# facebookresearch/SlowFast

Measured on NVIDIA H100. Metric: clips/sec (fwd+bwd) SlowFast-8x8-R50, higher is better.
Workload: dtype bf16x3-split operands, f32 accumulate/storage

## Files before the change

slowfast_b200/csrc/conv_stem.cu:

```cuda
#include <algorithm>
#include <cstdint>
#include <cstring>
#include <cuda_bf16.h>

#include "../../include/slowfast_b200.h"
#include "ptx.cuh"
#include "tmap.h"

namespace sfb {

constexpr int ST_MAX_STAGES = 8;
constexpr int ST_SEG_STRIDE = 2304;
constexpr int ST_SEG_PIX = 136;
constexpr int ST_WSEG_STRIDE = 1152;
constexpr int ST_WSEG_PIX = 72;
constexpr int ST_MMA_WARPS = 8;
constexpr int ST_FPROP_THREADS = 32 * (ST_MMA_WARPS + 1 + 4);
constexpr int ST_WGRAD_THREADS = 32 * (4 + 1);
constexpr int ST_BN_MAX = 128;
constexpr int ST_NPG_MAX = 4;

__device__ __forceinline__ void tma_load_5d(void* smem, const CUtensorMap* tm, uint64_t* bar, int32_t c0, int32_t c1,
                                            int32_t c2, int32_t c3, int32_t c4) {
  asm volatile(
      "cp.async.bulk.tensor.5d.shared::cluster.global.mbarrier::complete_tx::bytes [%0], [%1, {%3, %4, %5, %6, %7}], "
      "[%2];" ::"r"(smem_u32(smem)),
      "l"(tm), "r"(smem_u32(bar)), "r"(c0), "r"(c1), "r"(c2), "r"(c3), "r"(c4)
      : "memory");
}
__device__ __forceinline__ void tma_load_3d_(void* smem, const CUtensorMap* tm, uint64_t* bar, int32_t c0, int32_t c1,
                                             int32_t c2) {
  asm volatile(
      "cp.async.bulk.tensor.3d.shared::cluster.global.mbarrier::complete_tx::bytes [%0], [%1, {%3, %4, %5}], [%2];"
      ::"r"(smem_u32(smem)), "l"(tm), "r"(smem_u32(bar)), "r"(c0), "r"(c1), "r"(c2)
      : "memory");
}

struct StemParams {
  CUtensorMap tmX[2];
  CUtensorMap tmB[2];
  int N, OT, OH, OW;
  int st, sh, pt, ph, pw;
  int KT, KH, KW;
  int pairs, pps, k_blocks;
  int cout, BN, w_tiles, m_tiles;
  int stages;
  uint32_t stage_bytes, a_plane_bytes, b_bytes;
  uint32_t acc_pitch, off_acc, off_staging, off_red, off_bars;
  float* out;
  float* stats;
  int npg, n_groups, co_tiles, ktot, kb_total, splits, kb_per_split, w_chunks;
  float* dw;
};

template <int NSPLIT>
__global__ void __launch_bounds__(ST_FPROP_THREADS, 1) stem_fprop_kernel(const __grid_constant__ StemParams p) {
  extern __shared__ uint8_t smem_raw[];
  uint8_t* smem = reinterpret_cast<uint8_t*>((reinterpret_cast<uintptr_t>(smem_raw) + 1023) & ~uintptr_t(1023));
  const int warp = threadIdx.x >> 5, lane = threadIdx.x & 31;
  uint64_t* full = reinterpret_cast<uint64_t*>(smem + p.off_bars);
  uint64_t* empty = full + ST_MAX_STAGES;
  uint64_t* tfull = empty + ST_MAX_STAGES;
  uint64_t* tempty = tfull + 1;
  float* acc_tile = reinterpret_cast<float*>(smem + p.off_acc);
  if (threadIdx.x == 0) {
    for (int s = 0; s < p.stages; ++s) {
      mbar_init(&full[s], 1);
      mbar_init(&empty[s], 32 * ST_MMA_WARPS);
    }
    mbar_init(tfull, 32 * ST_MMA_WARPS);
    mbar_init(tempty, 4);
    fence_mbar_init();
    fence_proxy_async_smem();
  }
  __syncthreads();
  constexpr uint32_t NP = NSPLIT == 3 ? 2u : 1u;
  const int total_tiles = p.m_tiles;
  const int ksteps_per_pair = p.KW / 2;

  if (warp == ST_MMA_WARPS) {
    int stage = 0;
    uint32_t phase = 0;
    for (int tile = blockIdx.x; tile < total_tiles; tile += gridDim.x) {
      const int wt = tile % p.w_tiles;
      int r = tile / p.w_tiles;
      const int oh = r % p.OH;
      r /= p.OH;
      const int ot = r % p.OT;
      const int n = r / p.OT;
      const int w0 = wt * 128 - p.pw;
      for (int kb = 0; kb < p.k_blocks; ++kb) {
        mbar_wait(&empty[stage], phase ^ 1);
        if (elect_one()) {
          const int pair0 = kb * p.pps;
          const int nq = min(p.pps, p.pairs - pair0);
          mbar_expect_tx(&full[stage], (uint32_t(nq) * ST_SEG_PIX * 16u + p.b_bytes) * NP);
          uint8_t* st = smem + size_t(stage) * p.stage_bytes;
          for (int qq = 0; qq < nq; ++qq) {
            const int pair = pair0 + qq;
            const int kt = pair / p.KH, kh = pair - kt * p.KH;
            const int h = oh * p.sh - p.ph + kh, t = ot * p.st - p.pt + kt;
            for (uint32_t pl = 0; pl < NP; ++pl)
              tma_load_5d(st + pl * p.a_plane_bytes + qq * ST_SEG_STRIDE, &p.tmX[pl], &full[stage], 0, w0, h, t, n);
          }
          for (uint32_t pl = 0; pl < NP; ++pl)
            tma_load_2d(st + NP * p.a_plane_bytes + pl * p.b_bytes, &p.tmB[pl], &full[stage], kb * 64, 0);
        }
        __syncwarp();
        if (++stage == p.stages) {
          stage = 0;
          phase ^= 1;
        }
      }
    }
  } else if (warp < ST_MMA_WARPS) {
    const int g = warp >> 2;
    float d[ST_BN_MAX / 2];
    int stage = 0;
    uint32_t phase = 0;
    int it = 0;
    for (int tile = blockIdx.x; tile < total_tiles; tile += gridDim.x, ++it) {
      int held = -1;
      for (int kb = 0; kb < p.k_blocks; ++kb) {
        mbar_wait(&full[stage], phase);
        wgmma_fence();
        const int nq = min(p.pps, p.pairs - kb * p.pps);
        const uint32_t a_base = smem_u32(smem + size_t(stage) * p.stage_bytes) + uint32_t(g) * 1024u;
        const uint32_t b_base = smem_u32(smem + size_t(stage) * p.stage_bytes) + NP * p.a_plane_bytes;
        int kstep = 0;
        for (int qq = 0; qq < nq; ++qq) {
          for (int j = 0; j < ksteps_per_pair; ++j, ++kstep) {
            const uint32_t aa = a_base + qq * ST_SEG_STRIDE + uint32_t(2 * j) * 16u;
            const uint64_t a_hi = make_smem_desc(aa, 16, 128, 0);
            const uint64_t b_hi = make_smem_desc(b_base + uint32_t(kstep) * 32u, 16, 1024, 2);
            const uint32_t acc_flag = (kb | kstep) != 0 ? 1u : 0u;
            if (NSPLIT == 3) {
              const uint64_t a_lo = make_smem_desc(aa + p.a_plane_bytes, 16, 128, 0);
              const uint64_t b_lo = make_smem_desc(b_base + p.b_bytes + uint32_t(kstep) * 32u, 16, 1024, 2);
              wgmma_bf16<ST_BN_MAX, 0, 0>(d, p.BN, a_lo, b_hi, acc_flag);
              wgmma_bf16<ST_BN_MAX, 0, 0>(d, p.BN, a_hi, b_lo, 1u);
              wgmma_bf16<ST_BN_MAX, 0, 0>(d, p.BN, a_hi, b_hi, 1u);
            } else {
              wgmma_bf16<ST_BN_MAX, 0, 0>(d, p.BN, a_hi, b_hi, acc_flag);
            }
          }
        }
        wgmma_commit();
        wgmma_wait<1>();
        if (held >= 0) mbar_arrive(&empty[held]);
        held = stage;
        if (++stage == p.stages) {
          stage = 0;
          phase ^= 1;
        }
      }
      wgmma_wait<0>();
      mbar_arrive(&empty[held]);
      mbar_wait(tempty, (it & 1) ^ 1);
      acc_store<ST_BN_MAX>(d, p.BN, acc_tile + size_t(g) * 64 * p.acc_pitch, int(p.acc_pitch));
      mbar_arrive(tfull);
    }
  } else {
    const int q = warp - (ST_MMA_WARPS + 1);
    float* stg = reinterpret_cast<float*>(smem + p.off_staging) + q * (32 * 33);
    float* red = reinterpret_cast<float*>(smem + p.off_red);
    const float* arow = acc_tile + size_t(q * 32 + lane) * p.acc_pitch;
    int it = 0;
    for (int tile = blockIdx.x; tile < total_tiles; tile += gridDim.x, ++it) {
      const int acc = it & 1;
      const int wt = tile % p.w_tiles;
      const int rowi = tile / p.w_tiles;
      const int ow = wt * 128 + q * 32 + lane;
      const bool rvalid = ow < p.OW;
      const uint32_t rmask = __ballot_sync(0xffffffffu, rvalid);
      float* red_w = red + ((size_t(acc) * 4 + q) * p.BN) * 2;
      mbar_wait(tfull, it & 1);
      for (int c0 = 0; c0 < p.BN; c0 += 32) {
        uint32_t v0[16], v1[16];
        acc_ld_x16(arow + c0, v0);
        const bool second = (c0 + 16) < p.BN;
        if (second) acc_ld_x16(arow + c0 + 16, v1);
        if (c0 + 32 >= p.BN) {
          __syncwarp();
          if (lane == 0) mbar_arrive(tempty);
        }
#pragma unroll
        for (int j = 0; j < 16; ++j) stg[lane * 33 + j] = rvalid ? __uint_as_float(v0[j]) : 0.f;
#pragma unroll
        for (int j = 0; j < 16; ++j) stg[lane * 33 + 16 + j] = (rvalid && second) ? __uint_as_float(v1[j]) : 0.f;
        __syncwarp();
        {
          const int cl = c0 + lane;
          const bool cvalid = cl < min(p.BN, p.cout);
          float* dst = p.out + (static_cast<long long>(rowi) * p.OW + wt * 128 + q * 32) * p.cout + cl;
          if (p.cout <= 16 && (p.cout & (p.cout - 1)) == 0 && p.BN <= 32) {
            const int W = p.cout;
            const int R = 32 / W;
            const int col = lane & (W - 1), rsub = lane / W;
            float s = 0.f, s2 = 0.f;
            float* d2 = p.out + (static_cast<long long>(rowi) * p.OW + wt * 128 + q * 32) * p.cout + col;
            for (int r0 = 0; r0 < 32; r0 += R) {
              const int r = r0 + rsub;
              const float y = stg[r * 33 + col];
              s += y;
              s2 = fmaf(y, y, s2);
              if ((rmask >> r) & 1u) d2[static_cast<long long>(r) * p.cout] = y;
            }
            for (int o = W; o < 32; o <<= 1) {
              s += __shfl_xor_sync(0xffffffffu, s, o);
              s2 += __shfl_xor_sync(0xffffffffu, s2, o);
            }
            if (p.stats != nullptr && lane < W) {
              red_w[lane * 2 + 0] = s;
              red_w[lane * 2 + 1] = s2;
            }
            if (p.stats != nullptr && lane >= W && lane < p.BN) {
              red_w[lane * 2 + 0] = 0.f;
              red_w[lane * 2 + 1] = 0.f;
            }
            __syncwarp();
            continue;
          }
          float s = 0.f, s2 = 0.f;
#pragma unroll 8
          for (int r = 0; r < 32; ++r) {
            const float y = stg[r * 33 + lane];
            s += y;
            s2 = fmaf(y, y, s2);
            if (((rmask >> r) & 1u) && cvalid) dst[static_cast<long long>(r) * p.cout] = y;
          }
          if (p.stats != nullptr && cl < p.BN) {
            red_w[cl * 2 + 0] = s;
            red_w[cl * 2 + 1] = s2;
          }
          __syncwarp();
        }
      }
      if (p.stats != nullptr) {
        named_bar_sync(1, 128);
        const float* rb = red + size_t(acc) * 4 * p.BN * 2;
        for (int cl = q * 32 + lane; cl < p.BN; cl += 128) {
          if (cl < p.cout) {
            float s = 0.f, s2 = 0.f;
#pragma unroll
            for (int w = 0; w < 4; ++w) {
              s += rb[(size_t(w) * p.BN + cl) * 2 + 0];
              s2 += rb[(size_t(w) * p.BN + cl) * 2 + 1];
            }
            p.stats[size_t(cl) * p.m_tiles + tile] = s;
            p.stats[(size_t(p.cout) + cl) * p.m_tiles + tile] = s2;
          }
        }
      }
    }
  }
}

__device__ __forceinline__ void st_red_add_v4(float* addr, float a, float b, float c, float d) {
  asm volatile("red.global.add.v4.f32 [%0], {%1, %2, %3, %4};" ::"l"(addr), "f"(a), "f"(b), "f"(c), "f"(d)
               : "memory");
}

template <int NSPLIT>
__global__ void __launch_bounds__(ST_WGRAD_THREADS, 1) stem_wgrad_kernel(const __grid_constant__ StemParams p) {
  extern __shared__ uint8_t smem_raw[];
  uint8_t* smem = reinterpret_cast<uint8_t*>((reinterpret_cast<uintptr_t>(smem_raw) + 1023) & ~uintptr_t(1023));
  const int warp = threadIdx.x >> 5, lane = threadIdx.x & 31;
  uint64_t* full = reinterpret_cast<uint64_t*>(smem + p.off_bars);
  uint64_t* empty = full + ST_MAX_STAGES;
  constexpr uint32_t NP = NSPLIT == 3 ? 2u : 1u;

  const int split = blockIdx.x % p.splits;
  const int grp = blockIdx.x / p.splits;
  const int kb0 = split * p.kb_per_split;
  const int kb1 = min(p.kb_total, kb0 + p.kb_per_split);
  const int pair_base = grp * p.npg;
  const int npairs = min(p.npg, p.pairs - pair_base);
  const int ncols_pair = p.KW * 8;

  if (threadIdx.x == 0) {
    for (int s = 0; s < p.stages; ++s) {
      mbar_init(&full[s], 1);
      mbar_init(&empty[s], 128);
    }
    fence_mbar_init();
    fence_proxy_async_smem();
  }
  __syncthreads();
  const uint32_t dy_plane = 8192;

  if (kb1 > kb0 && npairs > 0) {
    if (warp == 4) {
      int stage = 0;
      uint32_t phase = 0;
      for (int kb = kb0; kb < kb1; ++kb) {
        mbar_wait(&empty[stage], phase ^ 1);
        if (elect_one()) {
          const int wc = kb % p.w_chunks;
          int r = kb / p.w_chunks;
          const int rowi = r;
          const int oh = r % p.OH;
          r /= p.OH;
          const int ot = r % p.OT;
          const int n = r / p.OT;
          const int ow0 = wc * 64;
          mbar_expect_tx(&full[stage], (dy_plane + uint32_t(npairs) * ST_WSEG_PIX * 16u) * NP);
          uint8_t* st = smem + size_t(stage) * p.stage_bytes;
          for (uint32_t pl = 0; pl < NP; ++pl) {
            tma_load_3d_(st + pl * dy_plane, &p.tmB[pl], &full[stage], 0, ow0, rowi);
            uint8_t* xb = st + NP * dy_plane + pl * p.a_plane_bytes;
            for (int j = 0; j < npairs; ++j) {
              const int pair = pair_base + j;
              const int kt = pair / p.KH, kh = pair - kt * p.KH;
              tma_load_5d(xb + j * ST_WSEG_STRIDE, &p.tmX[pl], &full[stage], 0, ow0 - p.pw, oh * p.sh - p.ph + kh,
                          ot * p.st - p.pt + kt, n);
            }
          }
        }
        __syncwarp();
        if (++stage == p.stages) {
          stage = 0;
          phase ^= 1;
        }
      }
    } else {
      float d[ST_NPG_MAX * 16];
      int stage = 0;
      uint32_t phase = 0;
      int held = -1;
      for (int kb = kb0; kb < kb1; ++kb) {
        mbar_wait(&full[stage], phase);
        wgmma_fence();
        const uint32_t a_base = smem_u32(smem + size_t(stage) * p.stage_bytes);
        const uint32_t x_base = a_base + NP * dy_plane;
#pragma unroll
        for (int j = 0; j < ST_NPG_MAX; ++j) {
          if (j < npairs) {
#pragma unroll
            for (int ks = 0; ks < 4; ++ks) {
              const uint64_t a_hi = make_smem_desc(a_base + ks * 2048, 0, 1024, 2);
              const uint64_t b_hi = make_smem_desc(x_base + j * ST_WSEG_STRIDE + ks * 256, 128, 16, 0);
              const uint32_t acc_flag = (kb != kb0 || ks != 0) ? 1u : 0u;
              if (NSPLIT == 3) {
                const uint64_t a_lo = make_smem_desc(a_base + dy_plane + ks * 2048, 0, 1024, 2);
                const uint64_t b_lo =
                    make_smem_desc(x_base + p.a_plane_bytes + j * ST_WSEG_STRIDE + ks * 256, 128, 16, 0);
                wgmma_bf16<32, 1, 1>(d + 16 * j, ncols_pair, a_lo, b_hi, acc_flag);
                wgmma_bf16<32, 1, 1>(d + 16 * j, ncols_pair, a_hi, b_lo, 1u);
                wgmma_bf16<32, 1, 1>(d + 16 * j, ncols_pair, a_hi, b_hi, 1u);
              } else {
                wgmma_bf16<32, 1, 1>(d + 16 * j, ncols_pair, a_hi, b_hi, acc_flag);
              }
            }
          }
        }
        wgmma_commit();
        wgmma_wait<1>();
        if (held >= 0) mbar_arrive(&empty[held]);
        held = stage;
        if (++stage == p.stages) {
          stage = 0;
          phase ^= 1;
        }
      }
      wgmma_wait<0>();
      const int co0 = warp * 16 + (lane >> 2);
      const int col_base = pair_base * ncols_pair;
#pragma unroll
      for (int j = 0; j < ST_NPG_MAX; ++j) {
        if (j < npairs) {
#pragma unroll
          for (int c = 0; c < 4; ++c) {
            if (8 * c < ncols_pair) {
#pragma unroll
              for (int h = 0; h < 2; ++h) {
                const int co = co0 + 8 * h;
                if (co < p.cout) {
                  float* dst = p.dw + size_t(co) * p.ktot + col_base + j * ncols_pair + 8 * c + 2 * (lane & 3);
                  asm volatile("red.global.add.v2.f32 [%0], {%1, %2};" ::"l"(dst), "f"(d[16 * j + 4 * c + 2 * h]),
                               "f"(d[16 * j + 4 * c + 2 * h + 1]) : "memory");
                }
              }
            }
          }
        }
      }
    }
  }
}

__global__ void stem_input_fold_kernel(const float* __restrict__ x, int n, int cin, int t, int h, int w,
                                       __nv_bfloat16* __restrict__ hi, __nv_bfloat16* __restrict__ lo) {
  const int w2 = w / 2;
  const int64_t thw = int64_t(t) * h * w;
  const int64_t items = int64_t(n) * t * h * w2;
  for (int64_t i = blockIdx.x * int64_t(blockDim.x) + threadIdx.x; i < items; i += int64_t(gridDim.x) * blockDim.x) {
    const int wp = int(i % w2);
    const int64_t rest = i / w2;
    const int64_t nt = rest / h;
    const int hh = int(rest - nt * h);
    const int64_t b = nt / t;
    const int tt = int(nt - b * t);
    float v[8];
#pragma unroll
    for (int j = 0; j < 8; ++j) v[j] = 0.f;
    for (int par = 0; par < 2; ++par)
      for (int c = 0; c < cin; ++c)
        v[par * cin + c] = x[(b * cin + c) * thw + (int64_t(tt) * h + hh) * w + 2 * wp + par];
    alignas(16) __nv_bfloat16 hv[8], lv[8];
#pragma unroll
    for (int j = 0; j < 8; ++j) {
      hv[j] = __float2bfloat16_rn(v[j]);
      lv[j] = __float2bfloat16_rn(v[j] - __bfloat162float(hv[j]));
    }
    *reinterpret_cast<uint4*>(hi + i * 8) = *reinterpret_cast<const uint4*>(hv);
    if (lo) *reinterpret_cast<uint4*>(lo + i * 8) = *reinterpret_cast<const uint4*>(lv);
  }
}

__global__ void stem_filter_fold_kernel(const float* __restrict__ w, float* __restrict__ dw, int cout, int cin, int kt,
                                        int kh, int kw, int pad, int kwf, __nv_bfloat16* __restrict__ hi,
                                        __nv_bfloat16* __restrict__ lo, const float* __restrict__ gmat, int reverse) {
  const int dmin = (-pad >= 0) ? (-pad) / 2 : -((pad + 1) / 2);
  const int64_t items = int64_t(cout) * kt * kh * kwf * 8;
  for (int64_t i = blockIdx.x * int64_t(blockDim.x) + threadIdx.x; i < items; i += int64_t(gridDim.x) * blockDim.x) {
    const int slot = int(i % 8);
    int64_t r = i / 8;
    const int kwp = int(r % kwf);
    r /= kwf;
    const int ih = int(r % kh);
    r /= kh;
    const int it = int(r % kt);
    const int co = int(r / kt);
    const int par = slot / cin, c = slot - par * cin;
    const int tap = 2 * (kwp + dmin) + par + pad;
    const bool valid = slot < 2 * cin && tap >= 0 && tap < kw;
    const int64_t widx = (((int64_t(co) * cin + c) * kt + it) * kh + ih) * kw + tap;
    if (reverse) {
      if (valid) dw[widx] = gmat[i];
    } else {
      const float v = valid ? w[widx] : 0.f;
      const __nv_bfloat16 h = __float2bfloat16_rn(v);
      hi[i] = h;
      if (lo) lo[i] = __float2bfloat16_rn(v - __bfloat162float(h));
    }
  }
}

typedef CUresult (*EncodeTiledFnS)(CUtensorMap*, CUtensorMapDataType, cuuint32_t, void*, const cuuint64_t*,
                                   const cuuint64_t*, const cuuint32_t*, const cuuint32_t*, CUtensorMapInterleave,
                                   CUtensorMapSwizzle, CUtensorMapL2promotion, CUtensorMapFloatOOBfill);
static EncodeTiledFnS st_encode() {
  static EncodeTiledFnS fn = nullptr;
  if (!fn) {
    cudaDriverEntryPointQueryResult q;
    void* f = nullptr;
    if (cudaGetDriverEntryPoint("cuTensorMapEncodeTiled", &f, cudaEnableDefault, &q) == cudaSuccess &&
        q == cudaDriverEntryPointSuccess)
      fn = reinterpret_cast<EncodeTiledFnS>(f);
  }
  return fn;
}
static int make_tmap_fold(CUtensorMap* out, const void* base, int n, int t, int h, int w2, uint32_t pix) {
  EncodeTiledFnS fn = st_encode();
  if (!fn) {
    set_error("cuTensorMapEncodeTiled entry point unavailable");
    return -1;
  }
  cuuint64_t dims[5] = {8, (cuuint64_t)w2, (cuuint64_t)h, (cuuint64_t)t, (cuuint64_t)n};
  cuuint64_t strides[4] = {16, 16ull * w2, 16ull * w2 * h, 16ull * w2 * h * t};
  cuuint32_t box[5] = {8, pix, 1, 1, 1};
  cuuint32_t estr[5] = {1, 1, 1, 1, 1};
  CUresult r = fn(out, CU_TENSOR_MAP_DATA_TYPE_BFLOAT16, 5, const_cast<void*>(base), dims, strides, box, estr,
                  CU_TENSOR_MAP_INTERLEAVE_NONE, CU_TENSOR_MAP_SWIZZLE_NONE, CU_TENSOR_MAP_L2_PROMOTION_L2_128B,
                  CU_TENSOR_MAP_FLOAT_OOB_FILL_NONE);
  if (r != CUDA_SUCCESS) {
    set_error("cuTensorMapEncodeTiled(fold 5d) failed (%d)", (int)r);
    return -2;
  }
  return 0;
}
static int make_tmap_dy3(CUtensorMap* out, const void* base, int64_t rows, int ow, int cout) {
  EncodeTiledFnS fn = st_encode();
  if (!fn) {
    set_error("cuTensorMapEncodeTiled entry point unavailable");
    return -1;
  }
  cuuint64_t dims[3] = {(cuuint64_t)cout, (cuuint64_t)ow, (cuuint64_t)rows};
  cuuint64_t strides[2] = {2ull * cout, 2ull * cout * ow};
  cuuint32_t box[3] = {64, 64, 1};
  cuuint32_t estr[3] = {1, 1, 1};
  CUresult r = fn(out, CU_TENSOR_MAP_DATA_TYPE_BFLOAT16, 3, const_cast<void*>(base), dims, strides, box, estr,
                  CU_TENSOR_MAP_INTERLEAVE_NONE, CU_TENSOR_MAP_SWIZZLE_128B, CU_TENSOR_MAP_L2_PROMOTION_L2_128B,
                  CU_TENSOR_MAP_FLOAT_OOB_FILL_NONE);
  if (r != CUDA_SUCCESS) {
    set_error("cuTensorMapEncodeTiled(dy 3d) failed (%d)", (int)r);
    return -2;
  }
  return 0;
}

static int st_sms = 0, st_smem = 0;
static int st_props() {
  if (st_sms) return 0;
  int dev = 0;
  if (cudaGetDevice(&dev) != cudaSuccess) {
    set_error("cudaGetDevice failed: no CUDA device");
    return -1;
  }
  cudaDeviceGetAttribute(&st_sms, cudaDevAttrMultiProcessorCount, dev);
  cudaDeviceGetAttribute(&st_smem, cudaDevAttrMaxSharedMemoryPerBlockOptin, dev);
  return 0;
}

static int fill_common(StemParams& p, const sfb_stem_desc* d) {
  if (d->kwf != 2 && d->kwf != 4) {
    set_error("sfb_stem: folded W taps must be 2 or 4 (got %d)", d->kwf);
    return -10;
  }
  if (d->cout % 8 || d->cout > 128) {
    set_error("sfb_stem: cout=%d must be a multiple of 8 and <= 128", d->cout);
    return -10;
  }
  p.N = d->n; p.OT = d->out_t; p.OH = d->out_h; p.OW = d->out_w;
  p.st = d->str_t; p.sh = d->str_h; p.pt = d->pad_t; p.ph = d->pad_h; p.pw = d->pad_wf;
  p.KT = d->kt; p.KH = d->kh; p.KW = d->kwf;
  p.pairs = d->kt * d->kh;
  p.cout = d->cout;
  p.ktot = p.pairs * d->kwf * 8;
  return 0;
}

}

using namespace sfb;
typedef __nv_bfloat16 bf16s;

extern "C" int sfb_stem_input_fold(const float* x, int32_t n, int32_t cin, int32_t t, int32_t h, int32_t w, void* hi,
                                   void* lo, void* stream) {
  if (cin < 1 || cin > 4 || (w & 1)) {
    set_error("sfb_stem_input_fold: cin=%d must be <= 4 and w=%d even", cin, w);
    return -10;
  }
  const int64_t items = int64_t(n) * t * h * (w / 2);
  int64_t grid = (items + 255) / 256;
  if (grid > 148 * 16) grid = 148 * 16;
  stem_input_fold_kernel<<<int(grid), 256, 0, (cudaStream_t)stream>>>(x, n, cin, t, h, w, (bf16s*)hi, (bf16s*)lo);
  cudaError_t e = cudaGetLastError();
  if (e != cudaSuccess) {
    set_error("sfb_stem_input_fold launch failed: %s", cudaGetErrorString(e));
    return -20;
  }
  return 0;
}

extern "C" int sfb_stem_filter_fold(const float* w, float* dw, int32_t cout, int32_t cin, int32_t kt, int32_t kh,
                                    int32_t kw, int32_t pad_w, int32_t kwf, void* hi, void* lo, const float* gmat,
                                    int32_t reverse, void* stream) {
  const int64_t items = int64_t(cout) * kt * kh * kwf * 8;
  int64_t grid = (items + 255) / 256;
  if (grid > 148 * 8) grid = 148 * 8;
  stem_filter_fold_kernel<<<int(grid), 256, 0, (cudaStream_t)stream>>>(w, dw, cout, cin, kt, kh, kw, pad_w, kwf,
                                                                       (bf16s*)hi, (bf16s*)lo, gmat, reverse);
  cudaError_t e = cudaGetLastError();
  if (e != cudaSuccess) {
    set_error("sfb_stem_filter_fold launch failed: %s", cudaGetErrorString(e));
    return -20;
  }
  return 0;
}

extern "C" int64_t sfb_stem_m_tiles(const sfb_stem_desc* d) {
  return int64_t(d->n) * d->out_t * d->out_h * ((d->out_w + 127) / 128);
}

extern "C" int sfb_stem_fprop(const sfb_stem_desc* d, void* stream_) {
  cudaStream_t stream = (cudaStream_t)stream_;
  if (st_props()) return -1;
  StemParams p;
  memset(&p, 0, sizeof(p));
  int rc = fill_common(p, d);
  if (rc) return rc;
  const int np = d->nsplit == 3 ? 2 : 1;
  p.pps = 64 / (d->kwf * 8);
  p.k_blocks = (p.pairs + p.pps - 1) / p.pps;
  p.BN = (d->cout + 15) / 16 * 16;
  if (p.BN > ST_BN_MAX) {
    set_error("sfb_stem_fprop: cout=%d > %d not supported", d->cout, ST_BN_MAX);
    return -10;
  }
  p.w_tiles = (d->out_w + 127) / 128;
  p.m_tiles = int(sfb_stem_m_tiles(d));
  p.a_plane_bytes = p.pps * ST_SEG_STRIDE;
  p.b_bytes = p.BN * 128;
  p.stage_bytes = ((p.a_plane_bytes + p.b_bytes) * np + 1023) / 1024 * 1024;
  p.a_plane_bytes = (p.a_plane_bytes + 1023) / 1024 * 1024;
  p.stage_bytes = (p.a_plane_bytes + p.b_bytes) * np;
  p.acc_pitch = uint32_t(p.BN) + 4;
  const uint32_t acc_bytes = 128u * p.acc_pitch * 4u;
  const uint32_t tail = acc_bytes + 4 * 32 * 33 * 4 + 2 * 4 * p.BN * 2 * 4 + 256;
  p.stages = std::min<int>(ST_MAX_STAGES, (uint32_t(st_smem) - 1024 - tail) / p.stage_bytes);
  p.stages = std::min(p.stages, std::max(2, p.k_blocks * 2));
  p.off_acc = p.stages * p.stage_bytes;
  p.off_staging = p.off_acc + acc_bytes;
  p.off_red = p.off_staging + 4 * 32 * 33 * 4;
  p.off_bars = p.off_red + 2 * 4 * p.BN * 2 * 4;
  const uint32_t smem_bytes = p.off_bars + 256 + 1024;
  p.out = d->out;
  p.stats = d->stats;
  for (int pl = 0; pl < np; ++pl) {
    rc = make_tmap_fold(&p.tmX[pl], pl ? d->x_lo : d->x_hi, d->n, d->t, d->h, d->wf, ST_SEG_PIX);
    if (rc) return rc;
    rc = make_tmap_2d_bf16(&p.tmB[pl], pl ? d->f_lo : d->f_hi, d->cout, p.ktot, p.ktot, p.BN, 64, SWZ_128);
    if (rc) return rc;
  }
  const int grid = std::min(p.m_tiles, st_sms);
  if (d->nsplit == 3) {
    static bool a = false;
    if (!a) { cudaFuncSetAttribute(stem_fprop_kernel<3>, cudaFuncAttributeMaxDynamicSharedMemorySize, st_smem); a = true; }
    stem_fprop_kernel<3><<<grid, ST_FPROP_THREADS, smem_bytes, stream>>>(p);
  } else {
    static bool a = false;
    if (!a) { cudaFuncSetAttribute(stem_fprop_kernel<1>, cudaFuncAttributeMaxDynamicSharedMemorySize, st_smem); a = true; }
    stem_fprop_kernel<1><<<grid, ST_FPROP_THREADS, smem_bytes, stream>>>(p);
  }
  cudaError_t e = cudaGetLastError();
  if (e != cudaSuccess) {
    set_error("sfb_stem_fprop launch failed: %s (smem=%u stages=%d)", cudaGetErrorString(e), smem_bytes, p.stages);
    return -20;
  }
  return 0;
}

extern "C" int sfb_stem_wgrad(const sfb_stem_desc* d, void* stream_) {
  cudaStream_t stream = (cudaStream_t)stream_;
  if (st_props()) return -1;
  if (d->cout > 64) {
    set_error("sfb_stem_wgrad: cout=%d > 64 not supported", d->cout);
    return -10;
  }
  StemParams p;
  memset(&p, 0, sizeof(p));
  int rc = fill_common(p, d);
  if (rc) return rc;
  const int np = d->nsplit == 3 ? 2 : 1;
  const int ncols_pair = d->kwf * 8;
  if (ncols_pair > 32) {
    set_error("sfb_stem_wgrad: %d folded W taps > 4 not supported", d->kwf);
    return -10;
  }
  p.npg = std::min(p.pairs, ST_NPG_MAX);
  p.n_groups = (p.pairs + p.npg - 1) / p.npg;
  p.w_chunks = (d->out_w + 63) / 64;
  p.kb_total = d->n * d->out_t * d->out_h * p.w_chunks;
  int splits = std::max(1, (2 * st_sms) / p.n_groups);
  splits = std::min(splits, std::max(1, p.kb_total / 8));
  p.kb_per_split = (p.kb_total + splits - 1) / splits;
  p.splits = (p.kb_total + p.kb_per_split - 1) / p.kb_per_split;
  p.a_plane_bytes = (p.npg * ST_WSEG_STRIDE + 127) / 128 * 128;
  p.stage_bytes = ((8192 + p.a_plane_bytes) * np + 1023) / 1024 * 1024;
  p.stages = std::min<int>(ST_MAX_STAGES, (uint32_t(st_smem) - 1024 - 256) / p.stage_bytes);
  p.stages = std::min(p.stages, std::max(2, p.kb_per_split));
  p.off_bars = p.stages * p.stage_bytes;
  const uint32_t smem_bytes = p.off_bars + 256 + 1024;
  p.dw = d->dwm;
  const int64_t rows = int64_t(d->n) * d->out_t * d->out_h;
  for (int pl = 0; pl < np; ++pl) {
    rc = make_tmap_fold(&p.tmX[pl], pl ? d->x_lo : d->x_hi, d->n, d->t, d->h, d->wf, ST_WSEG_PIX);
    if (rc) return rc;
    rc = make_tmap_dy3(&p.tmB[pl], pl ? d->dy_lo : d->dy_hi, rows, d->out_w, d->cout);
    if (rc) return rc;
  }
  const int grid = p.n_groups * p.splits;
  if (d->nsplit == 3) {
    static bool a = false;
    if (!a) { cudaFuncSetAttribute(stem_wgrad_kernel<3>, cudaFuncAttributeMaxDynamicSharedMemorySize, st_smem); a = true; }
    stem_wgrad_kernel<3><<<grid, ST_WGRAD_THREADS, smem_bytes, stream>>>(p);
  } else {
    static bool a = false;
    if (!a) { cudaFuncSetAttribute(stem_wgrad_kernel<1>, cudaFuncAttributeMaxDynamicSharedMemorySize, st_smem); a = true; }
    stem_wgrad_kernel<1><<<grid, ST_WGRAD_THREADS, smem_bytes, stream>>>(p);
  }
  cudaError_t e = cudaGetLastError();
  if (e != cudaSuccess) {
    set_error("sfb_stem_wgrad launch failed: %s (grid=%d smem=%u)", cudaGetErrorString(e), grid, smem_bytes);
    return -20;
  }
  return 0;
}

namespace sfb {
constexpr int SD_COUT = 8, SD_CIN = 3, SD_THREADS = 256, SD_TPT = 3;
struct StemDirectParams {
  const float* x;
  const __nv_bfloat16* dy_hi; const __nv_bfloat16* dy_lo;
  float* dw;
  int n, T, H, W, OT, OH, OW, KT, KH, KW, pt, ph, pw;
  int xw;
  int rows_total, rows_per_block;
};
__global__ void __launch_bounds__(SD_THREADS) stem_wgrad_direct_kernel(const StemDirectParams p) {
  extern __shared__ float sm[];
  float* xs = sm;
  float* dys = sm + size_t(p.KT) * p.KH * SD_CIN * p.xw;
  const int taps = SD_CIN * p.KT * p.KH * p.KW;
  int toff[SD_TPT], tkw[SD_TPT];
  bool tok[SD_TPT];
#pragma unroll
  for (int j = 0; j < SD_TPT; ++j) {
    const int tap = threadIdx.x + j * SD_THREADS;
    tok[j] = tap < taps;
    const int tt = tok[j] ? tap : 0;
    const int kw = tt % p.KW;
    int r = tt / p.KW;
    const int kh = r % p.KH;
    r /= p.KH;
    const int kt = r % p.KT;
    const int ci = r / p.KT;
    toff[j] = ((kt * p.KH + kh) * SD_CIN + ci) * p.xw + kw;
    tkw[j] = kw;
  }
  float acc[SD_TPT][SD_COUT];
#pragma unroll
  for (int j = 0; j < SD_TPT; ++j)
#pragma unroll
    for (int c = 0; c < SD_COUT; ++c) acc[j][c] = 0.f;
  const int r0 = blockIdx.x * p.rows_per_block;
  const int r1 = min(p.rows_total, r0 + p.rows_per_block);
  const int xrows = p.KT * p.KH * SD_CIN;
  const int w4 = p.W / 4;
  for (int row = r0; row < r1; ++row) {
    const int oh = row % p.OH;
    int r = row / p.OH;
    const int ot = r % p.OT;
    const int n = r / p.OT;
    __syncthreads();
    for (int i = threadIdx.x; i < xrows * (p.xw / 4); i += SD_THREADS) {
      const int q = i % (p.xw / 4);
      int rr = i / (p.xw / 4);
      const int ci = rr % SD_CIN;
      rr /= SD_CIN;
      const int kh = rr % p.KH;
      const int kt = rr / p.KH;
      const int it = ot - p.pt + kt, ih = oh * 2 - p.ph + kh;
      float4 v = make_float4(0.f, 0.f, 0.f, 0.f);
      const int wq = q - 1;
      if (it >= 0 && it < p.T && ih >= 0 && ih < p.H && wq >= 0 && wq < w4)
        v = *reinterpret_cast<const float4*>(p.x + (((int64_t(n) * SD_CIN + ci) * p.T + it) * p.H + ih) * p.W + wq * 4);
      *reinterpret_cast<float4*>(xs + ((kt * p.KH + kh) * SD_CIN + ci) * p.xw + q * 4) = v;
    }
    for (int i = threadIdx.x; i < p.OW * 2; i += SD_THREADS) {
      const int64_t off = (int64_t(row) * p.OW) * SD_COUT + i * 4;
      const uint2 h = *reinterpret_cast<const uint2*>(p.dy_hi + off);
      float4 v = make_float4(__uint_as_float(h.x << 16), __uint_as_float(h.x & 0xffff0000u), __uint_as_float(h.y << 16),
                             __uint_as_float(h.y & 0xffff0000u));
      if (p.dy_lo) {
        const uint2 l = *reinterpret_cast<const uint2*>(p.dy_lo + off);
        v.x += __uint_as_float(l.x << 16); v.y += __uint_as_float(l.x & 0xffff0000u);
        v.z += __uint_as_float(l.y << 16); v.w += __uint_as_float(l.y & 0xffff0000u);
      }
      *reinterpret_cast<float4*>(dys + i * 4) = v;
    }
    __syncthreads();
    const int cbase = 4 - p.pw;
#pragma unroll 4
    for (int ow = 0; ow < p.OW; ++ow) {
      const float4 d0 = *reinterpret_cast<const float4*>(dys + ow * 8);
      const float4 d1 = *reinterpret_cast<const float4*>(dys + ow * 8 + 4);
#pragma unroll
      for (int j = 0; j < SD_TPT; ++j) {
        const float xv = xs[toff[j] + cbase + 2 * ow];
        acc[j][0] = fmaf(d0.x, xv, acc[j][0]); acc[j][1] = fmaf(d0.y, xv, acc[j][1]);
        acc[j][2] = fmaf(d0.z, xv, acc[j][2]); acc[j][3] = fmaf(d0.w, xv, acc[j][3]);
        acc[j][4] = fmaf(d1.x, xv, acc[j][4]); acc[j][5] = fmaf(d1.y, xv, acc[j][5]);
        acc[j][6] = fmaf(d1.z, xv, acc[j][6]); acc[j][7] = fmaf(d1.w, xv, acc[j][7]);
      }
    }
  }
  (void)tkw;
#pragma unroll
  for (int j = 0; j < SD_TPT; ++j) {
    if (!tok[j]) continue;
    const int tap = threadIdx.x + j * SD_THREADS;
#pragma unroll
    for (int c = 0; c < SD_COUT; ++c) atomicAdd(p.dw + size_t(c) * taps + tap, acc[j][c]);
  }
}
}

extern "C" int sfb_stem_wgrad_direct(const float* x, int32_t n, int32_t cin, int32_t t, int32_t h, int32_t w,
                                     const void* dy_hi, const void* dy_lo, int32_t cout, int32_t kt, int32_t kh,
                                     int32_t kw, int32_t st, int32_t sh, int32_t sw, int32_t pt, int32_t ph, int32_t pw,
                                     float* dw, void* stream) {
  using namespace sfb;
  if (cin != SD_CIN || cout != SD_COUT || st != 1 || sh != 2 || sw != 2 || pw > 4 || w % 4 ||
      cin * kt * kh * kw > SD_THREADS * SD_TPT) {
    set_error("sfb_stem_wgrad_direct: only the 3 -> 8 channel, stride (1,2,2) stem with <= %d taps is supported",
              SD_THREADS * SD_TPT);
    return -10;
  }
  StemDirectParams p;
  p.x = x; p.dy_hi = (const __nv_bfloat16*)dy_hi; p.dy_lo = (const __nv_bfloat16*)dy_lo; p.dw = dw;
  p.n = n; p.T = t; p.H = h; p.W = w;
  p.OT = (t + 2 * pt - kt) / st + 1; p.OH = (h + 2 * ph - kh) / sh + 1; p.OW = (w + 2 * pw - kw) / sw + 1;
  p.KT = kt; p.KH = kh; p.KW = kw; p.pt = pt; p.ph = ph; p.pw = pw;
  const int need = 4 - pw + 2 * (p.OW - 1) + kw;
  p.xw = (std::max(need, w + 4) + 3) / 4 * 4 + 4;
  p.rows_total = n * p.OT * p.OH;
  int blocks = 148 * 2;
  if (blocks > p.rows_total) blocks = p.rows_total;
  p.rows_per_block = (p.rows_total + blocks - 1) / blocks;
  blocks = (p.rows_total + p.rows_per_block - 1) / p.rows_per_block;
  const size_t smem = (size_t(kt) * kh * SD_CIN * p.xw + size_t(p.OW) * SD_COUT) * sizeof(float);
  static bool attr = false;
  if (!attr) {
    cudaFuncSetAttribute(stem_wgrad_direct_kernel, cudaFuncAttributeMaxDynamicSharedMemorySize, 220 * 1024);
    attr = true;
  }
  cudaStream_t s = (cudaStream_t)stream;
  cudaMemsetAsync(dw, 0, size_t(cout) * cin * kt * kh * kw * sizeof(float), s);
  stem_wgrad_direct_kernel<<<blocks, SD_THREADS, smem, s>>>(p);
  cudaError_t e = cudaGetLastError();
  if (e != cudaSuccess) {
    set_error("sfb_stem_wgrad_direct launch failed: %s (smem=%zu)", cudaGetErrorString(e), smem);
    return -20;
  }
  return 0;
}
```

slowfast_b200/csrc/conv_stem8.cu:

```cuda
#include <algorithm>
#include <cstdint>
#include <cstring>
#include <cuda_bf16.h>

#include "../../include/slowfast_b200.h"
#include "ptx.cuh"
#include "tmap.h"

namespace sfb {

constexpr int T8_ROWS = 8;
constexpr int T8_SLOTS = 11;
constexpr int T8_KSTEPS = 6;
constexpr int T8_FPROP_THREADS = 32 * (8 + 1);
constexpr int T8_WGRAD_THREADS = 32 * (16 + 1);

__device__ __forceinline__ void t8_tma_5d(void* smem, const CUtensorMap* tm, uint64_t* bar, int32_t c0, int32_t c1,
                                          int32_t c2, int32_t c3, int32_t c4) {
  asm volatile(
      "cp.async.bulk.tensor.5d.shared::cluster.global.mbarrier::complete_tx::bytes [%0], [%1, {%3, %4, %5, %6, %7}], "
      "[%2];" ::"r"(smem_u32(smem)),
      "l"(tm), "r"(smem_u32(bar)), "r"(c0), "r"(c1), "r"(c2), "r"(c3), "r"(c4)
      : "memory");
}

struct Stem8Params {
  CUtensorMap tmX[2];
  CUtensorMap tmB[2];
  int N, T, OT, OH, OW, MR;
  int KT, pt, bands, tiles;
  uint32_t ab;
  uint32_t a_plane, a_bytes, b_plane, stage_bytes, off_red, off_bars;
  uint32_t zg;
  float* out;
  float* stats;
  int m_tiles;
  int splits0, splits1;
  int kt_groups, steps;
  float* dwm;
  int kfold;
};

template <int NSPLIT>
__global__ void __launch_bounds__(T8_FPROP_THREADS, 1) stem8_fprop_kernel(const __grid_constant__ Stem8Params p) {
  extern __shared__ uint8_t smem_raw[];
  uint8_t* smem = reinterpret_cast<uint8_t*>((reinterpret_cast<uintptr_t>(smem_raw) + 1023) & ~uintptr_t(1023));
  const int warp = threadIdx.x >> 5, lane = threadIdx.x & 31;
  uint64_t* full = reinterpret_cast<uint64_t*>(smem + p.off_bars);
  uint64_t* empty = full + 2;
  constexpr uint32_t NP = NSPLIT == 3 ? 2u : 1u;
  if (threadIdx.x == 0) {
    for (int s = 0; s < 2; ++s) {
      mbar_init(&full[s], 1);
      mbar_init(&empty[s], 256);
    }
    fence_mbar_init();
    fence_proxy_async_smem();
  }
  __syncthreads();

  if (warp == 8) {
    int stage = 0;
    uint32_t phase = 0;
    for (int tile = blockIdx.x; tile < p.tiles; tile += gridDim.x) {
      const int band = tile % p.bands;
      int r = tile / p.bands;
      const int ot = r % p.OT;
      const int n = r / p.OT;
      const int oh0 = band * T8_ROWS;
      const int kt_lo = max(0, p.pt - ot), kt_hi = min(p.KT, p.T + p.pt - ot);
      for (int kt = kt_lo; kt < kt_hi; ++kt) {
        mbar_wait(&empty[stage], phase ^ 1);
        if (elect_one()) {
          const int tin = ot + kt - p.pt;
          mbar_expect_tx(&full[stage], NP * (16u * uint32_t(T8_SLOTS * p.MR * 16) + p.b_plane));
          uint8_t* st = smem + size_t(stage) * p.stage_bytes;
          for (uint32_t pl = 0; pl < NP; ++pl) {
            for (int cls = 0; cls < 2; ++cls) {
              const int h2 = oh0 - 1 - cls;
              for (int j = 0; j < 8; ++j)
                t8_tma_5d(st + pl * p.a_plane + (cls * 8 + j) * p.ab, &p.tmX[pl], &full[stage], 0, j, h2, 2 * tin + cls, n);
            }
            tma_load_2d(st + p.a_bytes + pl * p.b_plane, &p.tmB[pl], &full[stage], 0, kt * int(p.zg));
          }
        }
        __syncwarp();
        if (++stage == 2) {
          stage = 0;
          phase ^= 1;
        }
      }
    }
  } else {
    const int g = warp >> 2;
    float* red = reinterpret_cast<float*>(smem + p.off_red);
    float d[32];
    int stage = 0;
    uint32_t phase = 0;
    int it = 0;
    for (int tile = blockIdx.x; tile < p.tiles; tile += gridDim.x, ++it) {
      const int band = tile % p.bands;
      const int rowg = tile / p.bands;
      const int ot = rowg % p.OT;
      const int kt_lo = max(0, p.pt - ot), kt_hi = min(p.KT, p.T + p.pt - ot);
      int held = -1;
      for (int kt = kt_lo; kt < kt_hi; ++kt) {
        mbar_wait(&full[stage], phase);
        wgmma_fence();
        const uint32_t a_base = smem_u32(smem + size_t(stage) * p.stage_bytes) + uint32_t(g) * 1024u;
        const uint32_t b_base = smem_u32(smem + size_t(stage) * p.stage_bytes) + p.a_bytes;
        for (int kh = 0; kh < 7; ++kh) {
          const int cls = (kh & 1) ^ 1;
          const int so = cls ? (kh >> 1) : ((kh - 1) >> 1);
#pragma unroll
          for (int i = 0; i < T8_KSTEPS; ++i) {
            const int arr = i < 4 ? 2 * i : 2 * i - 8;
            const int shift = i < 4 ? 0 : 1;
            const uint32_t aa = a_base + uint32_t(cls * 8 + arr) * p.ab + uint32_t(so * p.MR + shift) * 16u;
            const uint32_t bb = b_base + uint32_t(kh * 12 + 1 + 2 * i) * 128u;
            const uint64_t a_hi = make_smem_desc(aa, p.ab, 128, 0);
            const uint64_t b_hi = make_smem_desc(bb, 128, 128, 0);
            const uint32_t acc_flag = (kt != kt_lo || kh != 0 || i != 0) ? 1u : 0u;
            if (NSPLIT == 3) {
              const uint64_t a_lo = make_smem_desc(aa + p.a_plane, p.ab, 128, 0);
              const uint64_t b_lo = make_smem_desc(bb + p.b_plane, 128, 128, 0);
              wgmma_m64n64<0, 0>(d, a_lo, b_hi, acc_flag);
              wgmma_m64n64<0, 0>(d, a_hi, b_lo, 1u);
              wgmma_m64n64<0, 0>(d, a_hi, b_hi, 1u);
            } else {
              wgmma_m64n64<0, 0>(d, a_hi, b_hi, acc_flag);
            }
          }
        }
        wgmma_commit();
        wgmma_wait<1>();
        if (held >= 0) mbar_arrive(&empty[held]);
        held = stage;
        if (++stage == 2) {
          stage = 0;
          phase ^= 1;
        }
      }
      wgmma_wait<0>();
      if (held >= 0) mbar_arrive(&empty[held]);
      const int cp = 2 * (lane & 3);
      float s[2] = {0.f, 0.f}, s2[2] = {0.f, 0.f};
#pragma unroll
      for (int h = 0; h < 2; ++h) {
        const int rr = g * 64 + (warp & 3) * 16 + (lane >> 2) + 8 * h;
        const int ohl = rr / p.MR, m = rr - ohl * p.MR;
        if (ohl < T8_ROWS && m < p.MR - 1) {
          float* dst = p.out + ((static_cast<long long>(rowg) * p.OH + band * T8_ROWS + ohl) * p.OW + 8 * m) * 8 + cp;
#pragma unroll
          for (int c = 0; c < 8; ++c) {
            const float y0 = d[4 * c + 2 * h], y1 = d[4 * c + 2 * h + 1];
            *reinterpret_cast<float2*>(dst + (7 - c) * 8) = make_float2(y0, y1);
            s[0] += y0; s[1] += y1;
            s2[0] = fmaf(y0, y0, s2[0]); s2[1] = fmaf(y1, y1, s2[1]);
          }
        }
      }
      if (p.stats != nullptr) {
#pragma unroll
        for (int c = 0; c < 2; ++c) {
#pragma unroll
          for (int o = 4; o <= 16; o <<= 1) {
            s[c] += __shfl_xor_sync(0xffffffffu, s[c], o);
            s2[c] += __shfl_xor_sync(0xffffffffu, s2[c], o);
          }
        }
        float* rw = red + ((it & 1) * 8 + warp) * 16;
        if (lane < 4) {
          rw[cp] = s[0]; rw[cp + 1] = s[1];
          rw[8 + cp] = s2[0]; rw[8 + cp + 1] = s2[1];
        }
        named_bar_sync(1, 256);
        if (warp == 0 && lane < 16) {
          const float* rb = red + (it & 1) * 8 * 16;
          float tot = 0.f;
#pragma unroll
          for (int w = 0; w < 8; ++w) tot += rb[w * 16 + lane];
          p.stats[size_t(lane) * p.m_tiles + tile] = tot;
        }
      }
    }
  }
}


__device__ __forceinline__ void t8_red_add_v4(float* addr, float a, float b, float c, float d) {
  asm volatile("red.global.add.v4.f32 [%0], {%1, %2, %3, %4};" ::"l"(addr), "f"(a), "f"(b), "f"(c), "f"(d)
               : "memory");
}

template <int NSPLIT>
__global__ void __launch_bounds__(T8_WGRAD_THREADS, 1) stem8_wgrad_kernel(const __grid_constant__ Stem8Params p) {
  extern __shared__ uint8_t smem_raw[];
  uint8_t* smem = reinterpret_cast<uint8_t*>((reinterpret_cast<uintptr_t>(smem_raw) + 1023) & ~uintptr_t(1023));
  const int warp = threadIdx.x >> 5, lane = threadIdx.x & 31;
  uint64_t* full = reinterpret_cast<uint64_t*>(smem + p.off_bars);
  uint64_t* empty = full + 2;
  constexpr uint32_t NP = NSPLIT == 3 ? 2u : 1u;
  constexpr uint32_t DY_TILE = 16384;

  const int per0 = p.kt_groups * p.splits0;
  int cls, ktg, split, nsplits;
  if (int(blockIdx.x) < per0) {
    cls = 0;
    ktg = blockIdx.x / p.splits0;
    split = blockIdx.x - ktg * p.splits0;
    nsplits = p.splits0;
  } else {
    const int b = blockIdx.x - per0;
    cls = 1;
    ktg = b / p.splits1;
    split = b - ktg * p.splits1;
    nsplits = p.splits1;
  }
  const int ntaps = cls ? 4 : 3;
  const int kta = 2 * ktg, ktb = 2 * ktg + 1;
  const bool has_b = ktb < p.KT;
  const int per = (p.steps + nsplits - 1) / nsplits;
  const int s0 = split * per, s1 = min(p.steps, s0 + per);

  {
    uint4* z = reinterpret_cast<uint4*>(smem);
    const uint32_t n16 = (2u * p.stage_bytes) / 16u;
    for (uint32_t i = threadIdx.x; i < n16; i += blockDim.x) z[i] = make_uint4(0, 0, 0, 0);
  }
  if (threadIdx.x == 0) {
    for (int s = 0; s < 2; ++s) {
      mbar_init(&full[s], 1);
      mbar_init(&empty[s], 512);
    }
    fence_mbar_init();
  }
  fence_proxy_async_smem();
  __syncthreads();
  const uint32_t x_bytes = NP * 8u * p.ab;

  if (s1 > s0) {
    if (warp == 16) {
      int stage = 0;
      uint32_t phase = 0;
      for (int step = s0; step < s1; ++step) {
        const int band = step % p.bands;
        int r = step / p.bands;
        const int tin = r % p.T;
        const int n = r / p.T;
        const int oh0 = band * T8_ROWS;
        mbar_wait(&empty[stage], phase ^ 1);
        if (elect_one()) {
          const uint32_t dyb = uint32_t(T8_ROWS * p.MR) * 128u;
          mbar_expect_tx(&full[stage], NP * (8u * uint32_t(T8_SLOTS * p.MR * 16) + (has_b ? 2u : 1u) * dyb));
          uint8_t* st = smem + size_t(stage) * p.stage_bytes;
          const int h2 = oh0 - 1 - cls;
          for (uint32_t pl = 0; pl < NP; ++pl) {
            for (int j = 0; j < 8; ++j)
              t8_tma_5d(st + (pl * 8 + j) * p.ab, &p.tmX[pl], &full[stage], 0, j, h2, 2 * tin + cls, n);
            uint8_t* dyd = st + x_bytes + pl * 2 * DY_TILE;
            t8_tma_5d(dyd, &p.tmB[pl], &full[stage], 0, 0, oh0, tin - kta + p.pt, n);
            if (has_b) t8_tma_5d(dyd + DY_TILE, &p.tmB[pl], &full[stage], 0, 0, oh0, tin - ktb + p.pt, n);
          }
        }
        __syncwarp();
        if (++stage == 2) {
          stage = 0;
          phase ^= 1;
        }
      }
    } else {
      const int wg = warp >> 2, g = wg & 1, th = wg >> 1;
      float d0[2][32], d1[2][16];
      int stage = 0;
      uint32_t phase = 0;
      int held = -1;
      for (int step = s0; step < s1; ++step) {
        mbar_wait(&full[stage], phase);
        wgmma_fence();
        const uint32_t x_base = smem_u32(smem + size_t(stage) * p.stage_bytes);
        const uint32_t lbo_a = has_b ? DY_TILE : 0u;
        const uint32_t dy_base = x_base + x_bytes + uint32_t(g) * lbo_a;
#pragma unroll
        for (int u = 0; u < 2; ++u) {
          const int tq = 2 * th + u;
          if (tq < ntaps) {
#pragma unroll
            for (int ks = 0; ks < 8; ++ks) {
              const uint32_t xa = x_base + uint32_t(tq * p.MR) * 16u + uint32_t(ks) * 256u;
              const uint64_t a_hi = make_smem_desc(dy_base + ks * 2048, lbo_a, 1024, 2);
              const uint64_t b0_hi = make_smem_desc(xa, 128, p.ab, 0);
              const uint64_t b1_hi = make_smem_desc(xa + 16u, 128, p.ab, 0);
              const uint32_t acc_flag = (step != s0 || ks != 0) ? 1u : 0u;
              if (NSPLIT == 3) {
                const uint64_t a_lo = make_smem_desc(dy_base + 2 * DY_TILE + ks * 2048, lbo_a, 1024, 2);
                const uint64_t b0_lo = make_smem_desc(xa + 8u * p.ab, 128, p.ab, 0);
                const uint64_t b1_lo = make_smem_desc(xa + 8u * p.ab + 16u, 128, p.ab, 0);
                wgmma_m64n64<1, 1>(d0[u], a_lo, b0_hi, acc_flag);
                wgmma_m64n64<1, 1>(d0[u], a_hi, b0_lo, 1u);
                wgmma_m64n64<1, 1>(d0[u], a_hi, b0_hi, 1u);
                wgmma_m64n32<1, 1>(d1[u], a_lo, b1_hi, acc_flag);
                wgmma_m64n32<1, 1>(d1[u], a_hi, b1_lo, 1u);
                wgmma_m64n32<1, 1>(d1[u], a_hi, b1_hi, 1u);
              } else {
                wgmma_m64n64<1, 1>(d0[u], a_hi, b0_hi, acc_flag);
                wgmma_m64n32<1, 1>(d1[u], a_hi, b1_hi, acc_flag);
              }
            }
          }
        }
        wgmma_commit();
        wgmma_wait<1>();
        if (held >= 0) mbar_arrive(&empty[held]);
        held = stage;
        if (++stage == 2) {
          stage = 0;
          phase ^= 1;
        }
      }
      wgmma_wait<0>();
      const int kt = g ? ktb : kta;
      if (kt < p.KT) {
        const int sl = 2 * (lane & 3);
#pragma unroll
        for (int u = 0; u < 2; ++u) {
          const int tq = 2 * th + u;
          if (tq < ntaps) {
            const int kh = cls ? 2 * tq : 2 * tq + 1;
#pragma unroll
            for (int h = 0; h < 2; ++h) {
              const int mu = (warp & 3) * 16 + (lane >> 2) + 8 * h;
              const int j = mu >> 3, co = mu & 7;
              float* dst = p.dwm + size_t(co) * p.kfold + size_t((kt * 7 + kh) * 4) * 8 + sl;
#pragma unroll
              for (int gi = 0; gi < 12; ++gi) {
                const int kwp = gi - j;
                if (kwp >= 0 && kwp < 4) {
                  const float y0 = gi < 8 ? d0[u][4 * gi + 2 * h] : d1[u][4 * (gi - 8) + 2 * h];
                  const float y1 = gi < 8 ? d0[u][4 * gi + 2 * h + 1] : d1[u][4 * (gi - 8) + 2 * h + 1];
                  asm volatile("red.global.add.v2.f32 [%0], {%1, %2};" ::"l"(dst + kwp * 8), "f"(y0), "f"(y1) : "memory");
                }
              }
            }
          }
        }
      }
    }
  }
}


__global__ void stem8_input_fold_kernel(const float* __restrict__ x, int n, int cin, int t, int h, int w, int mr,
                                        __nv_bfloat16* __restrict__ hi, __nv_bfloat16* __restrict__ lo) {
  const int w2 = w / 2, gpr = 8 * mr, h2n = h / 2;
  const int64_t thw = int64_t(t) * h * w;
  const int64_t items = int64_t(n) * t * h * gpr;
  for (int64_t i = blockIdx.x * int64_t(blockDim.x) + threadIdx.x; i < items; i += int64_t(gridDim.x) * blockDim.x) {
    const int pp = int(i % gpr);
    const int64_t rest = i / gpr;
    const int64_t nt = rest / h;
    const int hh = int(rest - nt * h);
    const int64_t b = nt / t;
    const int tt = int(nt - b * t);
    const int pair = pp - 2;
    float v[8];
#pragma unroll
    for (int j = 0; j < 8; ++j) v[j] = 0.f;
    if (pair >= 0 && pair < w2)
      for (int par = 0; par < 2; ++par)
        for (int c = 0; c < cin; ++c)
          v[par * cin + c] = x[(b * cin + c) * thw + (int64_t(tt) * h + hh) * w + 2 * pair + par];
    alignas(16) __nv_bfloat16 hv[8], lv[8];
#pragma unroll
    for (int j = 0; j < 8; ++j) {
      hv[j] = __float2bfloat16_rn(v[j]);
      lv[j] = __float2bfloat16_rn(v[j] - __bfloat162float(hv[j]));
    }
    const int64_t row = ((b * 2 * t + 2 * tt + (hh & 1)) * h2n + (hh >> 1));
    const int64_t g = (row * 8 + (pp & 7)) * mr + (pp >> 3);
    *reinterpret_cast<uint4*>(hi + g * 8) = *reinterpret_cast<const uint4*>(hv);
    if (lo) *reinterpret_cast<uint4*>(lo + g * 8) = *reinterpret_cast<const uint4*>(lv);
  }
}

__global__ void stem8_filter_fold_kernel(const float* __restrict__ w, int cin, int kt, int zg,
                                         __nv_bfloat16* __restrict__ hi, __nv_bfloat16* __restrict__ lo) {
  const int items = kt * zg * 64;
  for (int i = blockIdx.x * blockDim.x + threadIdx.x; i < items; i += gridDim.x * blockDim.x) {
    const int slot = i & 7, co = (i >> 3) & 7;
    const int g = (i >> 6) % zg, it = (i >> 6) / zg;
    float v = 0.f;
    const int gi = g - 8;
    if (gi >= 0 && (gi % 12) < 4 && gi / 12 < 7 && slot < 2 * cin) {
      const int kh = gi / 12, kwp = gi % 12;
      const int par = slot / cin, c = slot - par * cin;
      const int tap = 2 * kwp + par - 1;
      if (tap >= 0 && tap < 7) v = w[(((int64_t(co) * cin + c) * kt + it) * 7 + kh) * 7 + tap];
    }
    const __nv_bfloat16 hb = __float2bfloat16_rn(v);
    hi[i] = hb;
    if (lo) lo[i] = __float2bfloat16_rn(v - __bfloat162float(hb));
  }
}

typedef CUresult (*EncodeTiledFn8)(CUtensorMap*, CUtensorMapDataType, cuuint32_t, void*, const cuuint64_t*,
                                   const cuuint64_t*, const cuuint32_t*, const cuuint32_t*, CUtensorMapInterleave,
                                   CUtensorMapSwizzle, CUtensorMapL2promotion, CUtensorMapFloatOOBfill);
static EncodeTiledFn8 t8_encode() {
  static EncodeTiledFn8 fn = nullptr;
  if (!fn) {
    cudaDriverEntryPointQueryResult q;
    void* f = nullptr;
    if (cudaGetDriverEntryPoint("cuTensorMapEncodeTiled", &f, cudaEnableDefault, &q) == cudaSuccess &&
        q == cudaDriverEntryPointSuccess)
      fn = reinterpret_cast<EncodeTiledFn8>(f);
  }
  return fn;
}
static int t8_tmap5(CUtensorMap* out, const void* base, const cuuint64_t dims[5], const cuuint64_t strides[4],
                    const cuuint32_t box[5], bool swz128, const char* what) {
  EncodeTiledFn8 fn = t8_encode();
  if (!fn) {
    set_error("cuTensorMapEncodeTiled entry point unavailable");
    return -1;
  }
  cuuint32_t estr[5] = {1, 1, 1, 1, 1};
  CUresult r = fn(out, CU_TENSOR_MAP_DATA_TYPE_BFLOAT16, 5, const_cast<void*>(base), dims, strides, box, estr,
                  CU_TENSOR_MAP_INTERLEAVE_NONE, swz128 ? CU_TENSOR_MAP_SWIZZLE_128B : CU_TENSOR_MAP_SWIZZLE_NONE,
                  CU_TENSOR_MAP_L2_PROMOTION_L2_128B, CU_TENSOR_MAP_FLOAT_OOB_FILL_NONE);
  if (r != CUDA_SUCCESS) {
    set_error("cuTensorMapEncodeTiled(%s) failed (%d)", what, (int)r);
    return -2;
  }
  return 0;
}

static int t8_sms = 0, t8_smem = 0;
static int t8_props() {
  if (t8_sms) return 0;
  int dev = 0;
  if (cudaGetDevice(&dev) != cudaSuccess) {
    set_error("cudaGetDevice failed: no CUDA device");
    return -1;
  }
  cudaDeviceGetAttribute(&t8_sms, cudaDevAttrMultiProcessorCount, dev);
  cudaDeviceGetAttribute(&t8_smem, cudaDevAttrMaxSharedMemoryPerBlockOptin, dev);
  return 0;
}

static bool t8_geometry_ok(const sfb_stem_desc* d) {
  return d->cout == 8 && d->kh == 7 && d->kwf == 4 && d->str_t == 1 && d->str_h == 2 && d->pad_h == 3 && d->pad_wf == 2 &&
         d->kt >= 1 && d->kt <= 8 && d->out_w % 8 == 0 && d->out_w >= 8 && d->out_w <= 120 && d->out_h % T8_ROWS == 0 &&
         d->h == 2 * d->out_h && d->wf == 8 * (d->out_w / 8 + 1) && d->out_t == d->t + 2 * d->pad_t - d->kt + 1;
}

static int t8_fill(Stem8Params& p, const sfb_stem_desc* d) {
  if (!t8_geometry_ok(d)) {
    set_error("sfb_stem8: unsupported geometry (cout=%d k=%dx%dx(%d folded) out=%dx%dx%d wf=%d)", d->cout, d->kt, d->kh,
              d->kwf, d->out_t, d->out_h, d->out_w, d->wf);
    return -10;
  }
  p.N = d->n; p.T = d->t; p.OT = d->out_t; p.OH = d->out_h; p.OW = d->out_w;
  p.MR = d->out_w / 8 + 1;
  p.KT = d->kt; p.pt = d->pad_t;
  p.bands = d->out_h / T8_ROWS;
  p.tiles = d->n * d->out_t * p.bands;
  p.m_tiles = p.tiles;
  p.ab = (uint32_t(T8_SLOTS * p.MR * 16) + 127u) / 128u * 128u;
  p.zg = 7 * 12 + 8;
  p.kfold = d->kt * 7 * 4 * 8;
  return 0;
}

static int t8_xmaps(Stem8Params& p, const sfb_stem_desc* d, int np) {
  const cuuint64_t row = 16ull * 8 * p.MR;
  cuuint64_t dims[5] = {(cuuint64_t)(8 * p.MR), 8, (cuuint64_t)(d->h / 2), (cuuint64_t)(2 * d->t), (cuuint64_t)d->n};
  cuuint64_t strides[4] = {16ull * p.MR, row, row * (d->h / 2), row * (d->h / 2) * 2 * d->t};
  cuuint32_t box[5] = {(cuuint32_t)(8 * p.MR), 1, (cuuint32_t)T8_SLOTS, 1, 1};
  for (int pl = 0; pl < np; ++pl) {
    int rc = t8_tmap5(&p.tmX[pl], pl ? d->x_lo : d->x_hi, dims, strides, box, false, "stem8 x");
    if (rc) return rc;
  }
  return 0;
}

}

using namespace sfb;
typedef __nv_bfloat16 bf16t;

extern "C" int sfb_stem8_supported(const sfb_stem_desc* d) { return t8_geometry_ok(d) ? 1 : 0; }

extern "C" int64_t sfb_stem8_m_tiles(const sfb_stem_desc* d) {
  return int64_t(d->n) * d->out_t * (d->out_h / T8_ROWS);
}

extern "C" int sfb_stem8_input_fold(const float* x, int32_t n, int32_t cin, int32_t t, int32_t h, int32_t w, void* hi,
                                    void* lo, void* stream) {
  if (cin < 1 || cin > 4 || (w % 16) || (h & 1)) {
    set_error("sfb_stem8_input_fold: cin=%d must be <= 4, w=%d a multiple of 16, h=%d even", cin, w, h);
    return -10;
  }
  const int mr = w / 16 + 1;
  const int64_t items = int64_t(n) * t * h * 8 * mr;
  int64_t grid = (items + 255) / 256;
  if (grid > 148 * 16) grid = 148 * 16;
  stem8_input_fold_kernel<<<int(grid), 256, 0, (cudaStream_t)stream>>>(x, n, cin, t, h, w, mr, (bf16t*)hi, (bf16t*)lo);
  cudaError_t e = cudaGetLastError();
  if (e != cudaSuccess) {
    set_error("sfb_stem8_input_fold launch failed: %s", cudaGetErrorString(e));
    return -20;
  }
  return 0;
}

extern "C" int sfb_stem8_filter_fold(const float* w, int32_t cin, int32_t kt, void* hi, void* lo, void* stream) {
  const int zg = 7 * 12 + 8;
  const int items = kt * zg * 64;
  stem8_filter_fold_kernel<<<(items + 255) / 256, 256, 0, (cudaStream_t)stream>>>(w, cin, kt, zg, (bf16t*)hi, (bf16t*)lo);
  cudaError_t e = cudaGetLastError();
  if (e != cudaSuccess) {
    set_error("sfb_stem8_filter_fold launch failed: %s", cudaGetErrorString(e));
    return -20;
  }
  return 0;
}

extern "C" int sfb_stem8_fprop(const sfb_stem_desc* d, void* stream_) {
  cudaStream_t stream = (cudaStream_t)stream_;
  if (t8_props()) return -1;
  Stem8Params p;
  memset(&p, 0, sizeof(p));
  int rc = t8_fill(p, d);
  if (rc) return rc;
  const int np = d->nsplit == 3 ? 2 : 1;
  p.a_plane = 16u * p.ab;
  p.a_bytes = np * p.a_plane;
  p.b_plane = p.zg * 128u;
  p.stage_bytes = (p.a_bytes + np * p.b_plane + 1023u) / 1024u * 1024u;
  p.off_red = 2 * p.stage_bytes;
  p.off_bars = p.off_red + 2 * 8 * 16 * 4;
  const uint32_t smem_bytes = p.off_bars + 128 + 1024;
  if (smem_bytes > uint32_t(t8_smem)) {
    set_error("sfb_stem8_fprop: %u bytes of shared memory needed, %d available", smem_bytes, t8_smem);
    return -11;
  }
  p.out = d->out;
  p.stats = d->stats;
  rc = t8_xmaps(p, d, np);
  if (rc) return rc;
  for (int pl = 0; pl < np; ++pl) {
    rc = make_tmap_2d_bf16(&p.tmB[pl], pl ? d->f_lo : d->f_hi, uint64_t(d->kt) * p.zg, 64, 64, p.zg, 64, SWZ_NONE);
    if (rc) return rc;
  }
  const int grid = std::min(p.tiles, t8_sms);
  if (d->nsplit == 3) {
    static bool a = false;
    if (!a) { cudaFuncSetAttribute(stem8_fprop_kernel<3>, cudaFuncAttributeMaxDynamicSharedMemorySize, t8_smem); a = true; }
    stem8_fprop_kernel<3><<<grid, T8_FPROP_THREADS, smem_bytes, stream>>>(p);
  } else {
    static bool a = false;
    if (!a) { cudaFuncSetAttribute(stem8_fprop_kernel<1>, cudaFuncAttributeMaxDynamicSharedMemorySize, t8_smem); a = true; }
    stem8_fprop_kernel<1><<<grid, T8_FPROP_THREADS, smem_bytes, stream>>>(p);
  }
  cudaError_t e = cudaGetLastError();
  if (e != cudaSuccess) {
    set_error("sfb_stem8_fprop launch failed: %s (smem=%u)", cudaGetErrorString(e), smem_bytes);
    return -20;
  }
  return 0;
}

extern "C" int sfb_stem8_wgrad(const sfb_stem_desc* d, void* stream_) {
  cudaStream_t stream = (cudaStream_t)stream_;
  if (t8_props()) return -1;
  Stem8Params p;
  memset(&p, 0, sizeof(p));
  int rc = t8_fill(p, d);
  if (rc) return rc;
  const int np = d->nsplit == 3 ? 2 : 1;
  p.stage_bytes = (np * 8u * p.ab + np * 2u * 16384u + 1023u) / 1024u * 1024u;
  if ((np * 8u * p.ab) % 1024u) {
    set_error("sfb_stem8_wgrad: operand arrays (%u bytes) do not keep the dY tiles 1024-byte aligned", np * 8u * p.ab);
    return -11;
  }
  p.off_bars = 2 * p.stage_bytes;
  const uint32_t smem_bytes = p.off_bars + 128 + 1024;
  if (smem_bytes > uint32_t(t8_smem)) {
    set_error("sfb_stem8_wgrad: %u bytes of shared memory needed, %d available", smem_bytes, t8_smem);
    return -11;
  }
  p.kt_groups = (d->kt + 1) / 2;
  p.steps = d->n * d->t * p.bands;
  const int per_group = std::max(2, t8_sms / p.kt_groups);
  p.splits1 = std::max(1, std::min(p.steps, (per_group * 4 + 3) / 7));
  p.splits0 = std::max(1, std::min(p.steps, per_group - p.splits1));
  p.dwm = d->dwm;
  rc = t8_xmaps(p, d, np);
  if (rc) return rc;
  {
    const cuuint64_t rowb = 16ull * d->out_w;
    cuuint64_t dims[5] = {64, (cuuint64_t)(d->out_w / 8), (cuuint64_t)d->out_h, (cuuint64_t)d->out_t, (cuuint64_t)d->n};
    cuuint64_t strides[4] = {128, rowb, rowb * d->out_h, rowb * d->out_h * d->out_t};
    cuuint32_t box[5] = {64, (cuuint32_t)p.MR, (cuuint32_t)T8_ROWS, 1, 1};
    for (int pl = 0; pl < np; ++pl) {
      rc = t8_tmap5(&p.tmB[pl], pl ? d->dy_lo : d->dy_hi, dims, strides, box, true, "stem8 dy");
      if (rc) return rc;
    }
  }
  const int grid = p.kt_groups * (p.splits0 + p.splits1);
  if (d->nsplit == 3) {
    static bool a = false;
    if (!a) { cudaFuncSetAttribute(stem8_wgrad_kernel<3>, cudaFuncAttributeMaxDynamicSharedMemorySize, t8_smem); a = true; }
    stem8_wgrad_kernel<3><<<grid, T8_WGRAD_THREADS, smem_bytes, stream>>>(p);
  } else {
    static bool a = false;
    if (!a) { cudaFuncSetAttribute(stem8_wgrad_kernel<1>, cudaFuncAttributeMaxDynamicSharedMemorySize, t8_smem); a = true; }
    stem8_wgrad_kernel<1><<<grid, T8_WGRAD_THREADS, smem_bytes, stream>>>(p);
  }
  cudaError_t e = cudaGetLastError();
  if (e != cudaSuccess) {
    set_error("sfb_stem8_wgrad launch failed: %s (grid=%d smem=%u)", cudaGetErrorString(e), grid, smem_bytes);
    return -20;
  }
  return 0;
}
```

Before: 174.4.

## Specialize stem conv kernels by width and taps, deepen pipelines, split wgrad work

The stem fprop kernel is now templated on output-channel width, so the wgmma shape and accumulator count match cout instead of a fixed 128. Tail pairs are handled with out-of-bounds TMA loads in place of runtime branches, and descriptor offsets are precomputed. The stem wgrad kernel now uses two warpgroups that split the K dimension and reduce through shared memory, templated on tap count and pairs per group. The stem8 kernels get a configurable pipeline depth (up to 4 stages), and stem8 wgrad launches one dY tile per kt instead of pairing taps. These changes target wasted MMA width, branch overhead and pipeline stalls, at the cost of more template instantiations and an extra smem reduction.

```diff
diff --git a/slowfast_b200/csrc/conv_stem.cu b/slowfast_b200/csrc/conv_stem.cu
--- a/slowfast_b200/csrc/conv_stem.cu
+++ b/slowfast_b200/csrc/conv_stem.cu
@@ -16,8 +16,9 @@
 constexpr int ST_WSEG_PIX = 72;
 constexpr int ST_MMA_WARPS = 8;
 constexpr int ST_FPROP_THREADS = 32 * (ST_MMA_WARPS + 1 + 4);
-constexpr int ST_WGRAD_THREADS = 32 * (4 + 1);
-constexpr int ST_BN_MAX = 128;
+constexpr int ST_WGRAD_THREADS = 32 * (ST_MMA_WARPS + 1);
+constexpr int ST_BN_MAX = 64;
+constexpr int ST_KSTEPS = 4;
 constexpr int ST_NPG_MAX = 4;
 
 __device__ __forceinline__ void tma_load_5d(void* smem, const CUtensorMap* tm, uint64_t* bar, int32_t c0, int32_t c1,
@@ -43,6 +44,7 @@
   int st, sh, pt, ph, pw;
   int KT, KH, KW;
   int pairs, pps, k_blocks;
+  uint32_t a_kstep[ST_KSTEPS];
   int cout, BN, w_tiles, m_tiles;
   int stages;
   uint32_t stage_bytes, a_plane_bytes, b_bytes;
@@ -53,7 +55,7 @@
   float* dw;
 };
 
-template <int NSPLIT>
+template <int NSPLIT, int BN>
 __global__ void __launch_bounds__(ST_FPROP_THREADS, 1) stem_fprop_kernel(const __grid_constant__ StemParams p) {
   extern __shared__ uint8_t smem_raw[];
   uint8_t* smem = reinterpret_cast<uint8_t*>((reinterpret_cast<uintptr_t>(smem_raw) + 1023) & ~uintptr_t(1023));
@@ -76,7 +78,6 @@
   __syncthreads();
   constexpr uint32_t NP = NSPLIT == 3 ? 2u : 1u;
   const int total_tiles = p.m_tiles;
-  const int ksteps_per_pair = p.KW / 2;
 
   if (warp == ST_MMA_WARPS) {
     int stage = 0;
@@ -93,13 +94,12 @@
         mbar_wait(&empty[stage], phase ^ 1);
         if (elect_one()) {
           const int pair0 = kb * p.pps;
-          const int nq = min(p.pps, p.pairs - pair0);
-          mbar_expect_tx(&full[stage], (uint32_t(nq) * ST_SEG_PIX * 16u + p.b_bytes) * NP);
+          mbar_expect_tx(&full[stage], (uint32_t(p.pps) * ST_SEG_PIX * 16u + p.b_bytes) * NP);
           uint8_t* st = smem + size_t(stage) * p.stage_bytes;
-          for (int qq = 0; qq < nq; ++qq) {
+          for (int qq = 0; qq < p.pps; ++qq) {
             const int pair = pair0 + qq;
             const int kt = pair / p.KH, kh = pair - kt * p.KH;
-            const int h = oh * p.sh - p.ph + kh, t = ot * p.st - p.pt + kt;
+            const int h = pair < p.pairs ? oh * p.sh - p.ph + kh : -1, t = ot * p.st - p.pt + kt;
             for (uint32_t pl = 0; pl < NP; ++pl)
               tma_load_5d(st + pl * p.a_plane_bytes + qq * ST_SEG_STRIDE, &p.tmX[pl], &full[stage], 0, w0, h, t, n);
           }
@@ -115,35 +115,32 @@
     }
   } else if (warp < ST_MMA_WARPS) {
     const int g = warp >> 2;
-    float d[ST_BN_MAX / 2];
+    float d[BN / 2];
     int stage = 0;
     uint32_t phase = 0;
     int it = 0;
     for (int tile = blockIdx.x; tile < total_tiles; tile += gridDim.x, ++it) {
+#pragma unroll
+      for (int i = 0; i < BN / 2; ++i) d[i] = 0.f;
       int held = -1;
       for (int kb = 0; kb < p.k_blocks; ++kb) {
         mbar_wait(&full[stage], phase);
         wgmma_fence();
-        const int nq = min(p.pps, p.pairs - kb * p.pps);
         const uint32_t a_base = smem_u32(smem + size_t(stage) * p.stage_bytes) + uint32_t(g) * 1024u;
         const uint32_t b_base = smem_u32(smem + size_t(stage) * p.stage_bytes) + NP * p.a_plane_bytes;
-        int kstep = 0;
-        for (int qq = 0; qq < nq; ++qq) {
-          for (int j = 0; j < ksteps_per_pair; ++j, ++kstep) {
-            const uint32_t aa = a_base + qq * ST_SEG_STRIDE + uint32_t(2 * j) * 16u;
-            const uint64_t a_hi = make_smem_desc(aa, 16, 128, 0);
-            const uint64_t b_hi = make_smem_desc(b_base + uint32_t(kstep) * 32u, 16, 1024, 2);
-            const uint32_t acc_flag = (kb | kstep) != 0 ? 1u : 0u;
-            if (NSPLIT == 3) {
-              const uint64_t a_lo = make_smem_desc(aa + p.a_plane_bytes, 16, 128, 0);
-              const uint64_t b_lo = make_smem_desc(b_base + p.b_bytes + uint32_t(kstep) * 32u, 16, 1024, 2);
-              wgmma_bf16<ST_BN_MAX, 0, 0>(d, p.BN, a_lo, b_hi, acc_flag);
-              wgmma_bf16<ST_BN_MAX, 0, 0>(d, p.BN, a_hi, b_lo, 1u);
-              wgmma_bf16<ST_BN_MAX, 0, 0>(d, p.BN, a_hi, b_hi, 1u);
-            } else {
-              wgmma_bf16<ST_BN_MAX, 0, 0>(d, p.BN, a_hi, b_hi, acc_flag);
-            }
+        const uint64_t a_hi0 = make_smem_desc(a_base, 16, 128, 0);
+        const uint64_t b_hi0 = make_smem_desc(b_base, 16, 1024, 2);
+#pragma unroll
+        for (int ks = 0; ks < ST_KSTEPS; ++ks) {
+          const uint64_t a_hi = a_hi0 + p.a_kstep[ks];
+          const uint64_t b_hi = b_hi0 + uint64_t(ks * 2);
+          if (NSPLIT == 3) {
+            const uint64_t a_lo = a_hi + (p.a_plane_bytes >> 4);
+            const uint64_t b_lo = b_hi + (p.b_bytes >> 4);
+            wgmma_m64n<BN>(d, a_lo, b_hi);
+            wgmma_m64n<BN>(d, a_hi, b_lo);
           }
+          wgmma_m64n<BN>(d, a_hi, b_hi);
         }
         wgmma_commit();
         wgmma_wait<1>();
@@ -157,7 +154,7 @@
       wgmma_wait<0>();
       mbar_arrive(&empty[held]);
       mbar_wait(tempty, (it & 1) ^ 1);
-      acc_store<ST_BN_MAX>(d, p.BN, acc_tile + size_t(g) * 64 * p.acc_pitch, int(p.acc_pitch));
+      acc_store<BN>(d, BN, acc_tile + size_t(g) * 64 * p.acc_pitch, int(p.acc_pitch));
       mbar_arrive(tfull);
     }
   } else {
@@ -261,7 +258,7 @@
                : "memory");
 }
 
-template <int NSPLIT>
+template <int NSPLIT, int KWF, int NPG>
 __global__ void __launch_bounds__(ST_WGRAD_THREADS, 1) stem_wgrad_kernel(const __grid_constant__ StemParams p) {
   extern __shared__ uint8_t smem_raw[];
   uint8_t* smem = reinterpret_cast<uint8_t*>((reinterpret_cast<uintptr_t>(smem_raw) + 1023) & ~uintptr_t(1023));
@@ -269,19 +266,20 @@
   uint64_t* full = reinterpret_cast<uint64_t*>(smem + p.off_bars);
   uint64_t* empty = full + ST_MAX_STAGES;
   constexpr uint32_t NP = NSPLIT == 3 ? 2u : 1u;
+  constexpr int NC = KWF * 8;
+  constexpr int NACC = NPG * NC / 2;
 
   const int split = blockIdx.x % p.splits;
   const int grp = blockIdx.x / p.splits;
   const int kb0 = split * p.kb_per_split;
   const int kb1 = min(p.kb_total, kb0 + p.kb_per_split);
-  const int pair_base = grp * p.npg;
-  const int npairs = min(p.npg, p.pairs - pair_base);
-  const int ncols_pair = p.KW * 8;
+  const int pair_base = grp * NPG;
+  const int npairs = min(NPG, p.pairs - pair_base);
 
   if (threadIdx.x == 0) {
     for (int s = 0; s < p.stages; ++s) {
       mbar_init(&full[s], 1);
-      mbar_init(&empty[s], 128);
+      mbar_init(&empty[s], 32 * ST_MMA_WARPS);
     }
     fence_mbar_init();
     fence_proxy_async_smem();
@@ -289,8 +287,8 @@
   __syncthreads();
   const uint32_t dy_plane = 8192;
 
-  if (kb1 > kb0 && npairs > 0) {
-    if (warp == 4) {
+  if (kb1 > kb0) {
+    if (warp == ST_MMA_WARPS) {
       int stage = 0;
       uint32_t phase = 0;
       for (int kb = kb0; kb < kb1; ++kb) {
@@ -304,16 +302,16 @@
           const int ot = r % p.OT;
           const int n = r / p.OT;
           const int ow0 = wc * 64;
-          mbar_expect_tx(&full[stage], (dy_plane + uint32_t(npairs) * ST_WSEG_PIX * 16u) * NP);
+          mbar_expect_tx(&full[stage], (dy_plane + uint32_t(NPG) * ST_WSEG_PIX * 16u) * NP);
           uint8_t* st = smem + size_t(stage) * p.stage_bytes;
           for (uint32_t pl = 0; pl < NP; ++pl) {
             tma_load_3d_(st + pl * dy_plane, &p.tmB[pl], &full[stage], 0, ow0, rowi);
             uint8_t* xb = st + NP * dy_plane + pl * p.a_plane_bytes;
-            for (int j = 0; j < npairs; ++j) {
+            for (int j = 0; j < NPG; ++j) {
               const int pair = pair_base + j;
               const int kt = pair / p.KH, kh = pair - kt * p.KH;
-              tma_load_5d(xb + j * ST_WSEG_STRIDE, &p.tmX[pl], &full[stage], 0, ow0 - p.pw, oh * p.sh - p.ph + kh,
-                          ot * p.st - p.pt + kt, n);
+              const int h = j < npairs ? oh * p.sh - p.ph + kh : -1;
+              tma_load_5d(xb + j * ST_WSEG_STRIDE, &p.tmX[pl], &full[stage], 0, ow0 - p.pw, h, ot * p.st - p.pt + kt, n);
             }
           }
         }
@@ -324,34 +322,31 @@
         }
       }
     } else {
-      float d[ST_NPG_MAX * 16];
+      const int g = warp >> 2;
+      float d[NACC];
+#pragma unroll
+      for (int i = 0; i < NACC; ++i) d[i] = 0.f;
       int stage = 0;
       uint32_t phase = 0;
       int held = -1;
       for (int kb = kb0; kb < kb1; ++kb) {
         mbar_wait(&full[stage], phase);
         wgmma_fence();
-        const uint32_t a_base = smem_u32(smem + size_t(stage) * p.stage_bytes);
-        const uint32_t x_base = a_base + NP * dy_plane;
-#pragma unroll
-        for (int j = 0; j < ST_NPG_MAX; ++j) {
-          if (j < npairs) {
-#pragma unroll
-            for (int ks = 0; ks < 4; ++ks) {
-              const uint64_t a_hi = make_smem_desc(a_base + ks * 2048, 0, 1024, 2);
-              const uint64_t b_hi = make_smem_desc(x_base + j * ST_WSEG_STRIDE + ks * 256, 128, 16, 0);
-              const uint32_t acc_flag = (kb != kb0 || ks != 0) ? 1u : 0u;
-              if (NSPLIT == 3) {
-                const uint64_t a_lo = make_smem_desc(a_base + dy_plane + ks * 2048, 0, 1024, 2);
-                const uint64_t b_lo =
-                    make_smem_desc(x_base + p.a_plane_bytes + j * ST_WSEG_STRIDE + ks * 256, 128, 16, 0);
-                wgmma_bf16<32, 1, 1>(d + 16 * j, ncols_pair, a_lo, b_hi, acc_flag);
-                wgmma_bf16<32, 1, 1>(d + 16 * j, ncols_pair, a_hi, b_lo, 1u);
-                wgmma_bf16<32, 1, 1>(d + 16 * j, ncols_pair, a_hi, b_hi, 1u);
-              } else {
-                wgmma_bf16<32, 1, 1>(d + 16 * j, ncols_pair, a_hi, b_hi, acc_flag);
-              }
+        const uint32_t a_base = smem_u32(smem + size_t(stage) * p.stage_bytes) + uint32_t(g) * 2u * 2048u;
+        const uint32_t x_base = smem_u32(smem + size_t(stage) * p.stage_bytes) + NP * dy_plane + uint32_t(g) * 2u * 256u;
+#pragma unroll
+        for (int j = 0; j < NPG; ++j) {
+#pragma unroll
+          for (int ks = 0; ks < 2; ++ks) {
+            const uint64_t a_hi = make_smem_desc(a_base + ks * 2048, 0, 1024, 2);
+            const uint64_t b_hi = make_smem_desc(x_base + j * ST_WSEG_STRIDE + ks * 256, 128, 16, 0);
+            if (NSPLIT == 3) {
+              const uint64_t a_lo = a_hi + (dy_plane >> 4);
+              const uint64_t b_lo = b_hi + (p.a_plane_bytes >> 4);
+              wgmma_m64n<NC, 1, 1>(d + j * (NC / 2), a_lo, b_hi);
+              wgmma_m64n<NC, 1, 1>(d + j * (NC / 2), a_hi, b_lo);
             }
+            wgmma_m64n<NC, 1, 1>(d + j * (NC / 2), a_hi, b_hi);
           }
         }
         wgmma_commit();
@@ -364,21 +359,31 @@
         }
       }
       wgmma_wait<0>();
-      const int co0 = warp * 16 + (lane >> 2);
-      const int col_base = pair_base * ncols_pair;
-#pragma unroll
-      for (int j = 0; j < ST_NPG_MAX; ++j) {
-        if (j < npairs) {
-#pragma unroll
-          for (int c = 0; c < 4; ++c) {
-            if (8 * c < ncols_pair) {
+      float* red = reinterpret_cast<float*>(smem);
+      const int t = threadIdx.x & 127;
+      named_bar_sync(1, 32 * ST_MMA_WARPS);
+      if (g == 1) {
+#pragma unroll
+        for (int i = 0; i < NACC; ++i) red[i * 128 + t] = d[i];
+      }
+      named_bar_sync(1, 32 * ST_MMA_WARPS);
+      if (g == 0) {
+#pragma unroll
+        for (int i = 0; i < NACC; ++i) d[i] += red[i * 128 + t];
+        const int co0 = warp * 16 + (lane >> 2);
+        const int col_base = pair_base * NC;
+#pragma unroll
+        for (int j = 0; j < NPG; ++j) {
+          if (j < npairs) {
+#pragma unroll
+            for (int c = 0; c < NC / 8; ++c) {
 #pragma unroll
               for (int h = 0; h < 2; ++h) {
                 const int co = co0 + 8 * h;
                 if (co < p.cout) {
-                  float* dst = p.dw + size_t(co) * p.ktot + col_base + j * ncols_pair + 8 * c + 2 * (lane & 3);
-                  asm volatile("red.global.add.v2.f32 [%0], {%1, %2};" ::"l"(dst), "f"(d[16 * j + 4 * c + 2 * h]),
-                               "f"(d[16 * j + 4 * c + 2 * h + 1]) : "memory");
+                  float* dst = p.dw + size_t(co) * p.ktot + col_base + j * NC + 8 * c + 2 * (lane & 3);
+                  asm volatile("red.global.add.v2.f32 [%0], {%1, %2};" ::"l"(dst), "f"(d[j * (NC / 2) + 4 * c + 2 * h]),
+                               "f"(d[j * (NC / 2) + 4 * c + 2 * h + 1]) : "memory");
                 }
               }
             }
@@ -584,6 +589,11 @@
   const int np = d->nsplit == 3 ? 2 : 1;
   p.pps = 64 / (d->kwf * 8);
   p.k_blocks = (p.pairs + p.pps - 1) / p.pps;
+  for (int ks = 0; ks < ST_KSTEPS; ++ks) {
+    const int per_pair = d->kwf / 2;
+    const int qq = ks / per_pair, j = ks % per_pair;
+    p.a_kstep[ks] = uint32_t(qq * ST_SEG_STRIDE + 2 * j * 16) >> 4;
+  }
   p.BN = (d->cout + 15) / 16 * 16;
   if (p.BN > ST_BN_MAX) {
     set_error("sfb_stem_fprop: cout=%d > %d not supported", d->cout, ST_BN_MAX);
@@ -615,14 +625,19 @@
     if (rc) return rc;
   }
   const int grid = std::min(p.m_tiles, st_sms);
-  if (d->nsplit == 3) {
-    static bool a = false;
-    if (!a) { cudaFuncSetAttribute(stem_fprop_kernel<3>, cudaFuncAttributeMaxDynamicSharedMemorySize, st_smem); a = true; }
-    stem_fprop_kernel<3><<<grid, ST_FPROP_THREADS, smem_bytes, stream>>>(p);
-  } else {
-    static bool a = false;
-    if (!a) { cudaFuncSetAttribute(stem_fprop_kernel<1>, cudaFuncAttributeMaxDynamicSharedMemorySize, st_smem); a = true; }
-    stem_fprop_kernel<1><<<grid, ST_FPROP_THREADS, smem_bytes, stream>>>(p);
+  {
+    typedef void (*KernelFn)(const StemParams);
+#define SFB_STEM_FNS(S) {stem_fprop_kernel<S, 16>, stem_fprop_kernel<S, 32>, stem_fprop_kernel<S, 48>, \
+                         stem_fprop_kernel<S, 64>}
+    static const KernelFn fns[2][ST_BN_MAX / 16] = {SFB_STEM_FNS(1), SFB_STEM_FNS(3)};
+#undef SFB_STEM_FNS
+    static bool attr[2][ST_BN_MAX / 16] = {};
+    const int a = d->nsplit == 3 ? 1 : 0, b = p.BN / 16 - 1;
+    if (!attr[a][b]) {
+      cudaFuncSetAttribute(fns[a][b], cudaFuncAttributeMaxDynamicSharedMemorySize, st_smem);
+      attr[a][b] = true;
+    }
+    fns[a][b]<<<grid, ST_FPROP_THREADS, smem_bytes, stream>>>(p);
   }
   cudaError_t e = cudaGetLastError();
   if (e != cudaSuccess) {
@@ -649,7 +664,7 @@
     set_error("sfb_stem_wgrad: %d folded W taps > 4 not supported", d->kwf);
     return -10;
   }
-  p.npg = std::min(p.pairs, ST_NPG_MAX);
+  p.npg = ((p.pairs + 2) / 3) * 3 < ((p.pairs + 3) / 4) * 4 ? 3 : ST_NPG_MAX;
   p.n_groups = (p.pairs + p.npg - 1) / p.npg;
   p.w_chunks = (d->out_w + 63) / 64;
   p.kb_total = d->n * d->out_t * d->out_h * p.w_chunks;
@@ -661,7 +676,7 @@
   p.stage_bytes = ((8192 + p.a_plane_bytes) * np + 1023) / 1024 * 1024;
   p.stages = std::min<int>(ST_MAX_STAGES, (uint32_t(st_smem) - 1024 - 256) / p.stage_bytes);
   p.stages = std::min(p.stages, std::max(2, p.kb_per_split));
-  p.off_bars = p.stages * p.stage_bytes;
+  p.off_bars = std::max(p.stages * p.stage_bytes, uint32_t(64 * p.npg * ncols_pair * 4));
   const uint32_t smem_bytes = p.off_bars + 256 + 1024;
   p.dw = d->dwm;
   const int64_t rows = int64_t(d->n) * d->out_t * d->out_h;
@@ -672,14 +687,19 @@
     if (rc) return rc;
   }
   const int grid = p.n_groups * p.splits;
-  if (d->nsplit == 3) {
-    static bool a = false;
-    if (!a) { cudaFuncSetAttribute(stem_wgrad_kernel<3>, cudaFuncAttributeMaxDynamicSharedMemorySize, st_smem); a = true; }
-    stem_wgrad_kernel<3><<<grid, ST_WGRAD_THREADS, smem_bytes, stream>>>(p);
-  } else {
-    static bool a = false;
-    if (!a) { cudaFuncSetAttribute(stem_wgrad_kernel<1>, cudaFuncAttributeMaxDynamicSharedMemorySize, st_smem); a = true; }
-    stem_wgrad_kernel<1><<<grid, ST_WGRAD_THREADS, smem_bytes, stream>>>(p);
+  {
+    typedef void (*KernelFn)(const StemParams);
+#define SFB_STEM_FNS(S) {stem_wgrad_kernel<S, 2, 3>, stem_wgrad_kernel<S, 2, 4>, stem_wgrad_kernel<S, 4, 3>, \
+                         stem_wgrad_kernel<S, 4, 4>}
+    static const KernelFn fns[2][4] = {SFB_STEM_FNS(1), SFB_STEM_FNS(3)};
+#undef SFB_STEM_FNS
+    static bool attr[2][4] = {};
+    const int a = d->nsplit == 3 ? 1 : 0, b = (d->kwf / 2 - 1) * 2 + (p.npg - 3);
+    if (!attr[a][b]) {
+      cudaFuncSetAttribute(fns[a][b], cudaFuncAttributeMaxDynamicSharedMemorySize, st_smem);
+      attr[a][b] = true;
+    }
+    fns[a][b]<<<grid, ST_WGRAD_THREADS, smem_bytes, stream>>>(p);
   }
   cudaError_t e = cudaGetLastError();
   if (e != cudaSuccess) {
diff --git a/slowfast_b200/csrc/conv_stem8.cu b/slowfast_b200/csrc/conv_stem8.cu
--- a/slowfast_b200/csrc/conv_stem8.cu
+++ b/slowfast_b200/csrc/conv_stem8.cu
@@ -12,6 +12,7 @@
 constexpr int T8_ROWS = 8;
 constexpr int T8_SLOTS = 11;
 constexpr int T8_KSTEPS = 6;
+constexpr int T8_MAX_STAGES = 4;
 constexpr int T8_FPROP_THREADS = 32 * (8 + 1);
 constexpr int T8_WGRAD_THREADS = 32 * (16 + 1);
 
@@ -29,6 +30,7 @@
   CUtensorMap tmB[2];
   int N, T, OT, OH, OW, MR;
   int KT, pt, bands, tiles;
+  int stages;
   uint32_t ab;
   uint32_t a_plane, a_bytes, b_plane, stage_bytes, off_red, off_bars;
   uint32_t zg;
@@ -36,7 +38,7 @@
   float* stats;
   int m_tiles;
   int splits0, splits1;
-  int kt_groups, steps;
+  int steps;
   float* dwm;
   int kfold;
 };
@@ -47,10 +49,10 @@
   uint8_t* smem = reinterpret_cast<uint8_t*>((reinterpret_cast<uintptr_t>(smem_raw) + 1023) & ~uintptr_t(1023));
   const int warp = threadIdx.x >> 5, lane = threadIdx.x & 31;
   uint64_t* full = reinterpret_cast<uint64_t*>(smem + p.off_bars);
-  uint64_t* empty = full + 2;
+  uint64_t* empty = full + T8_MAX_STAGES;
   constexpr uint32_t NP = NSPLIT == 3 ? 2u : 1u;
   if (threadIdx.x == 0) {
-    for (int s = 0; s < 2; ++s) {
+    for (int s = 0; s < p.stages; ++s) {
       mbar_init(&full[s], 1);
       mbar_init(&empty[s], 256);
     }
@@ -85,7 +87,7 @@
           }
         }
         __syncwarp();
-        if (++stage == 2) {
+        if (++stage == p.stages) {
           stage = 0;
           phase ^= 1;
         }
@@ -103,12 +105,15 @@
       const int rowg = tile / p.bands;
       const int ot = rowg % p.OT;
       const int kt_lo = max(0, p.pt - ot), kt_hi = min(p.KT, p.T + p.pt - ot);
+#pragma unroll
+      for (int i = 0; i < 32; ++i) d[i] = 0.f;
       int held = -1;
       for (int kt = kt_lo; kt < kt_hi; ++kt) {
         mbar_wait(&full[stage], phase);
         wgmma_fence();
         const uint32_t a_base = smem_u32(smem + size_t(stage) * p.stage_bytes) + uint32_t(g) * 1024u;
         const uint32_t b_base = smem_u32(smem + size_t(stage) * p.stage_bytes) + p.a_bytes;
+#pragma unroll
         for (int kh = 0; kh < 7; ++kh) {
           const int cls = (kh & 1) ^ 1;
           const int so = cls ? (kh >> 1) : ((kh - 1) >> 1);
@@ -120,23 +125,20 @@
             const uint32_t bb = b_base + uint32_t(kh * 12 + 1 + 2 * i) * 128u;
             const uint64_t a_hi = make_smem_desc(aa, p.ab, 128, 0);
             const uint64_t b_hi = make_smem_desc(bb, 128, 128, 0);
-            const uint32_t acc_flag = (kt != kt_lo || kh != 0 || i != 0) ? 1u : 0u;
             if (NSPLIT == 3) {
-              const uint64_t a_lo = make_smem_desc(aa + p.a_plane, p.ab, 128, 0);
-              const uint64_t b_lo = make_smem_desc(bb + p.b_plane, 128, 128, 0);
-              wgmma_m64n64<0, 0>(d, a_lo, b_hi, acc_flag);
+              const uint64_t a_lo = a_hi + (p.a_plane >> 4);
+              const uint64_t b_lo = b_hi + (p.b_plane >> 4);
+              wgmma_m64n64<0, 0>(d, a_lo, b_hi, 1u);
               wgmma_m64n64<0, 0>(d, a_hi, b_lo, 1u);
-              wgmma_m64n64<0, 0>(d, a_hi, b_hi, 1u);
-            } else {
-              wgmma_m64n64<0, 0>(d, a_hi, b_hi, acc_flag);
             }
+            wgmma_m64n64<0, 0>(d, a_hi, b_hi, 1u);
           }
         }
         wgmma_commit();
         wgmma_wait<1>();
         if (held >= 0) mbar_arrive(&empty[held]);
         held = stage;
-        if (++stage == 2) {
+        if (++stage == p.stages) {
           stage = 0;
           phase ^= 1;
         }
@@ -193,45 +195,44 @@
                : "memory");
 }
 
+constexpr uint32_t T8_DY_TILE = 16384;
+
 template <int NSPLIT>
 __global__ void __launch_bounds__(T8_WGRAD_THREADS, 1) stem8_wgrad_kernel(const __grid_constant__ Stem8Params p) {
   extern __shared__ uint8_t smem_raw[];
   uint8_t* smem = reinterpret_cast<uint8_t*>((reinterpret_cast<uintptr_t>(smem_raw) + 1023) & ~uintptr_t(1023));
   const int warp = threadIdx.x >> 5, lane = threadIdx.x & 31;
   uint64_t* full = reinterpret_cast<uint64_t*>(smem + p.off_bars);
-  uint64_t* empty = full + 2;
+  uint64_t* empty = full + T8_MAX_STAGES;
   constexpr uint32_t NP = NSPLIT == 3 ? 2u : 1u;
-  constexpr uint32_t DY_TILE = 16384;
-
-  const int per0 = p.kt_groups * p.splits0;
-  int cls, ktg, split, nsplits;
+
+  const int per0 = p.KT * p.splits0;
+  int cls, kt, split, nsplits;
   if (int(blockIdx.x) < per0) {
     cls = 0;
-    ktg = blockIdx.x / p.splits0;
-    split = blockIdx.x - ktg * p.splits0;
+    kt = blockIdx.x / p.splits0;
+    split = blockIdx.x - kt * p.splits0;
     nsplits = p.splits0;
   } else {
     const int b = blockIdx.x - per0;
     cls = 1;
-    ktg = b / p.splits1;
-    split = b - ktg * p.splits1;
+    kt = b / p.splits1;
+    split = b - kt * p.splits1;
     nsplits = p.splits1;
   }
   const int ntaps = cls ? 4 : 3;
-  const int kta = 2 * ktg, ktb = 2 * ktg + 1;
-  const bool has_b = ktb < p.KT;
   const int per = (p.steps + nsplits - 1) / nsplits;
   const int s0 = split * per, s1 = min(p.steps, s0 + per);
 
   {
     uint4* z = reinterpret_cast<uint4*>(smem);
-    const uint32_t n16 = (2u * p.stage_bytes) / 16u;
+    const uint32_t n16 = (uint32_t(p.stages) * p.stage_bytes) / 16u;
     for (uint32_t i = threadIdx.x; i < n16; i += blockDim.x) z[i] = make_uint4(0, 0, 0, 0);
   }
   if (threadIdx.x == 0) {
-    for (int s = 0; s < 2; ++s) {
+    for (int s = 0; s < p.stages; ++s) {
       mbar_init(&full[s], 1);
-      mbar_init(&empty[s], 512);
+      mbar_init(&empty[s], 128 * ntaps);
     }
     fence_mbar_init();
   }
@@ -252,26 +253,28 @@
         mbar_wait(&empty[stage], phase ^ 1);
         if (elect_one()) {
           const uint32_t dyb = uint32_t(T8_ROWS * p.MR) * 128u;
-          mbar_expect_tx(&full[stage], NP * (8u * uint32_t(T8_SLOTS * p.MR * 16) + (has_b ? 2u : 1u) * dyb));
+          mbar_expect_tx(&full[stage], NP * (8u * uint32_t(T8_SLOTS * p.MR * 16) + dyb));
           uint8_t* st = smem + size_t(stage) * p.stage_bytes;
           const int h2 = oh0 - 1 - cls;
           for (uint32_t pl = 0; pl < NP; ++pl) {
             for (int j = 0; j < 8; ++j)
               t8_tma_5d(st + (pl * 8 + j) * p.ab, &p.tmX[pl], &full[stage], 0, j, h2, 2 * tin + cls, n);
-            uint8_t* dyd = st + x_bytes + pl * 2 * DY_TILE;
-            t8_tma_5d(dyd, &p.tmB[pl], &full[stage], 0, 0, oh0, tin - kta + p.pt, n);
-            if (has_b) t8_tma_5d(dyd + DY_TILE, &p.tmB[pl], &full[stage], 0, 0, oh0, tin - ktb + p.pt, n);
+            t8_tma_5d(st + x_bytes + pl * T8_DY_TILE, &p.tmB[pl], &full[stage], 0, 0, oh0, tin - kt + p.pt, n);
           }
         }
         __syncwarp();
-        if (++stage == 2) {
+        if (++stage == p.stages) {
           stage = 0;
           phase ^= 1;
         }
       }
-    } else {
-      const int wg = warp >> 2, g = wg & 1, th = wg >> 1;
-      float d0[2][32], d1[2][16];
+    } else if ((warp >> 2) < ntaps) {
+      const int tq = warp >> 2;
+      float d0[32], d1[16];
+#pragma unroll
+      for (int i = 0; i < 32; ++i) d0[i] = 0.f;
+#pragma unroll
+      for (int i = 0; i < 16; ++i) d1[i] = 0.f;
       int stage = 0;
       uint32_t phase = 0;
       int held = -1;
@@ -279,69 +282,49 @@
         mbar_wait(&full[stage], phase);
         wgmma_fence();
         const uint32_t x_base = smem_u32(smem + size_t(stage) * p.stage_bytes);
-        const uint32_t lbo_a = has_b ? DY_TILE : 0u;
-        const uint32_t dy_base = x_base + x_bytes + uint32_t(g) * lbo_a;
-#pragma unroll
-        for (int u = 0; u < 2; ++u) {
-          const int tq = 2 * th + u;
-          if (tq < ntaps) {
-#pragma unroll
-            for (int ks = 0; ks < 8; ++ks) {
-              const uint32_t xa = x_base + uint32_t(tq * p.MR) * 16u + uint32_t(ks) * 256u;
-              const uint64_t a_hi = make_smem_desc(dy_base + ks * 2048, lbo_a, 1024, 2);
-              const uint64_t b0_hi = make_smem_desc(xa, 128, p.ab, 0);
-              const uint64_t b1_hi = make_smem_desc(xa + 16u, 128, p.ab, 0);
-              const uint32_t acc_flag = (step != s0 || ks != 0) ? 1u : 0u;
-              if (NSPLIT == 3) {
-                const uint64_t a_lo = make_smem_desc(dy_base + 2 * DY_TILE + ks * 2048, lbo_a, 1024, 2);
-                const uint64_t b0_lo = make_smem_desc(xa + 8u * p.ab, 128, p.ab, 0);
-                const uint64_t b1_lo = make_smem_desc(xa + 8u * p.ab + 16u, 128, p.ab, 0);
-                wgmma_m64n64<1, 1>(d0[u], a_lo, b0_hi, acc_flag);
-                wgmma_m64n64<1, 1>(d0[u], a_hi, b0_lo, 1u);
-                wgmma_m64n64<1, 1>(d0[u], a_hi, b0_hi, 1u);
-                wgmma_m64n32<1, 1>(d1[u], a_lo, b1_hi, acc_flag);
-                wgmma_m64n32<1, 1>(d1[u], a_hi, b1_lo, 1u);
-                wgmma_m64n32<1, 1>(d1[u], a_hi, b1_hi, 1u);
-              } else {
-                wgmma_m64n64<1, 1>(d0[u], a_hi, b0_hi, acc_flag);
-                wgmma_m64n32<1, 1>(d1[u], a_hi, b1_hi, acc_flag);
-              }
-            }
+        const uint32_t dy_base = x_base + x_bytes;
+#pragma unroll
+        for (int ks = 0; ks < 8; ++ks) {
+          const uint32_t xa = x_base + uint32_t(tq * p.MR) * 16u + uint32_t(ks) * 256u;
+          const uint64_t a_hi = make_smem_desc(dy_base + ks * 2048, 0, 1024, 2);
+          const uint64_t b0_hi = make_smem_desc(xa, 128, p.ab, 0);
+          const uint64_t b1_hi = b0_hi + 1;
+          if (NSPLIT == 3) {
+            const uint64_t a_lo = a_hi + (T8_DY_TILE >> 4);
+            const uint64_t b0_lo = b0_hi + ((8u * p.ab) >> 4);
+            const uint64_t b1_lo = b0_lo + 1;
+            wgmma_m64n64<1, 1>(d0, a_lo, b0_hi, 1u);
+            wgmma_m64n64<1, 1>(d0, a_hi, b0_lo, 1u);
+            wgmma_m64n32<1, 1>(d1, a_lo, b1_hi, 1u);
+            wgmma_m64n32<1, 1>(d1, a_hi, b1_lo, 1u);
           }
+          wgmma_m64n64<1, 1>(d0, a_hi, b0_hi, 1u);
+          wgmma_m64n32<1, 1>(d1, a_hi, b1_hi, 1u);
         }
         wgmma_commit();
         wgmma_wait<1>();
         if (held >= 0) mbar_arrive(&empty[held]);
         held = stage;
-        if (++stage == 2) {
+        if (++stage == p.stages) {
           stage = 0;
           phase ^= 1;
         }
       }
       wgmma_wait<0>();
-      const int kt = g ? ktb : kta;
-      if (kt < p.KT) {
-        const int sl = 2 * (lane & 3);
-#pragma unroll
-        for (int u = 0; u < 2; ++u) {
-          const int tq = 2 * th + u;
-          if (tq < ntaps) {
-            const int kh = cls ? 2 * tq : 2 * tq + 1;
-#pragma unroll
-            for (int h = 0; h < 2; ++h) {
-              const int mu = (warp & 3) * 16 + (lane >> 2) + 8 * h;
-              const int j = mu >> 3, co = mu & 7;
-              float* dst = p.dwm + size_t(co) * p.kfold + size_t((kt * 7 + kh) * 4) * 8 + sl;
-#pragma unroll
-              for (int gi = 0; gi < 12; ++gi) {
-                const int kwp = gi - j;
-                if (kwp >= 0 && kwp < 4) {
-                  const float y0 = gi < 8 ? d0[u][4 * gi + 2 * h] : d1[u][4 * (gi - 8) + 2 * h];
-                  const float y1 = gi < 8 ? d0[u][4 * gi + 2 * h + 1] : d1[u][4 * (gi - 8) + 2 * h + 1];
-                  asm volatile("red.global.add.v2.f32 [%0], {%1, %2};" ::"l"(dst + kwp * 8), "f"(y0), "f"(y1) : "memory");
-                }
-              }
-            }
+      const int kh = cls ? 2 * tq : 2 * tq + 1;
+      const int sl = 2 * (lane & 3);
+#pragma unroll
+      for (int h = 0; h < 2; ++h) {
+        const int mu = (warp & 3) * 16 + (lane >> 2) + 8 * h;
+        const int j = mu >> 3, co = mu & 7;
+        float* dst = p.dwm + size_t(co) * p.kfold + size_t((kt * 7 + kh) * 4) * 8 + sl;
+#pragma unroll
+        for (int gi = 0; gi < 12; ++gi) {
+          const int kwp = gi - j;
+          if (kwp >= 0 && kwp < 4) {
+            const float y0 = gi < 8 ? d0[4 * gi + 2 * h] : d1[4 * (gi - 8) + 2 * h];
+            const float y1 = gi < 8 ? d0[4 * gi + 2 * h + 1] : d1[4 * (gi - 8) + 2 * h + 1];
+            asm volatile("red.global.add.v2.f32 [%0], {%1, %2};" ::"l"(dst + kwp * 8), "f"(y0), "f"(y1) : "memory");
           }
         }
       }
@@ -538,7 +521,9 @@
   p.a_bytes = np * p.a_plane;
   p.b_plane = p.zg * 128u;
   p.stage_bytes = (p.a_bytes + np * p.b_plane + 1023u) / 1024u * 1024u;
-  p.off_red = 2 * p.stage_bytes;
+  const uint32_t tail = 2 * 8 * 16 * 4 + 128 + 1024;
+  p.stages = std::max(2, std::min<int>(T8_MAX_STAGES, (uint32_t(t8_smem) - tail) / p.stage_bytes));
+  p.off_red = p.stages * p.stage_bytes;
   p.off_bars = p.off_red + 2 * 8 * 16 * 4;
   const uint32_t smem_bytes = p.off_bars + 128 + 1024;
   if (smem_bytes > uint32_t(t8_smem)) {
@@ -579,20 +564,20 @@
   int rc = t8_fill(p, d);
   if (rc) return rc;
   const int np = d->nsplit == 3 ? 2 : 1;
-  p.stage_bytes = (np * 8u * p.ab + np * 2u * 16384u + 1023u) / 1024u * 1024u;
+  p.stage_bytes = (np * 8u * p.ab + np * T8_DY_TILE + 1023u) / 1024u * 1024u;
   if ((np * 8u * p.ab) % 1024u) {
     set_error("sfb_stem8_wgrad: operand arrays (%u bytes) do not keep the dY tiles 1024-byte aligned", np * 8u * p.ab);
     return -11;
   }
-  p.off_bars = 2 * p.stage_bytes;
+  p.stages = std::max(2, std::min<int>(T8_MAX_STAGES, (uint32_t(t8_smem) - 128 - 1024) / p.stage_bytes));
+  p.off_bars = p.stages * p.stage_bytes;
   const uint32_t smem_bytes = p.off_bars + 128 + 1024;
   if (smem_bytes > uint32_t(t8_smem)) {
     set_error("sfb_stem8_wgrad: %u bytes of shared memory needed, %d available", smem_bytes, t8_smem);
     return -11;
   }
-  p.kt_groups = (d->kt + 1) / 2;
   p.steps = d->n * d->t * p.bands;
-  const int per_group = std::max(2, t8_sms / p.kt_groups);
+  const int per_group = std::max(2, t8_sms / p.KT);
   p.splits1 = std::max(1, std::min(p.steps, (per_group * 4 + 3) / 7));
   p.splits0 = std::max(1, std::min(p.steps, per_group - p.splits1));
   p.dwm = d->dwm;
@@ -608,7 +593,7 @@
       if (rc) return rc;
     }
   }
-  const int grid = p.kt_groups * (p.splits0 + p.splits1);
+  const int grid = p.KT * (p.splits0 + p.splits1);
   if (d->nsplit == 3) {
     static bool a = false;
     if (!a) { cudaFuncSetAttribute(stem8_wgrad_kernel<3>, cudaFuncAttributeMaxDynamicSharedMemorySize, t8_smem); a = true; }
```

After: 180.2, median of 6. +3.4%, better.
